# davide-gurrieri/parallel-GCN

Hardware: AMD Instinct MI355X
Metric: training epochs/sec (2-layer GCN, hidden=16) on reddit (higher is better)
Workload: dtype fp32

## Files before the change

include/pgcn.h:

```cpp
#ifndef PGCN_H
#define PGCN_H
#include <stddef.h>
#include <stdint.h>

#ifdef __cplusplus
extern "C" {
#endif

#define PGCN_OK 0
#define PGCN_E_INVALID (-1)
#define PGCN_E_NOMEM (-2)
#define PGCN_E_IO (-3)
#define PGCN_E_COMM (-4)
#define PGCN_E_NODEVICE (-5)

const char *pgcn_status_string(int status);
int pgcn_version(void);


void pgcn_rng_seed(uint64_t state[2]);
void pgcn_rng_seed_glibc(unsigned int seed, uint64_t state[2]);
void pgcn_rng_jump(uint64_t state[2], uint64_t k);

typedef struct pgcn_graph pgcn_graph;
// ... 227 lines not shown
#define PGCN_CKPT_ATTENTION 8
int pgcn_checkpoint_attention(const char *path, int *heads, float *dropout);
#define PGCN_CKPT_SAGE 16
int pgcn_checkpoint_sage(const char *path, int *aggregator, int *root_weight);
#define PGCN_CKPT_READOUT 32
int pgcn_checkpoint_readout(const char *path, int *mode, int *num_graphs);
#define PGCN_CKPT_LINKS 64
int pgcn_checkpoint_links(const char *path, int *decoder, long long *num_pairs);
int pgcn_params_sizeof(void);
long long pgcn_gcn_predict(pgcn_gcn *g, int *cls, float *conf, float *probs);
int pgcn_gcn_confusion(pgcn_gcn *g, int split, long long *counts);
long long pgcn_gcn_predict_multilabel(pgcn_gcn *g, uint32_t *bits, float *probs);
int pgcn_gcn_multilabel_counts(pgcn_gcn *g, int split, long long *counts);
long long pgcn_gcn_predict_links(pgcn_gcn *g, float *scores, float *probs);
int pgcn_gcn_link_counts(pgcn_gcn *g, int split, long long *counts);
int pgcn_gcn_score_pairs(pgcn_gcn *g, const int *src, const int *dst, long long m, float *scores);
int pgcn_gcn_profile(pgcn_gcn *g, int enable);
int pgcn_gcn_profile_read(pgcn_gcn *g, double *graphsum_ms_total, long long *graphsum_calls,
                          double *graphsum_bytes_total);
int pgcn_gcn_profile_read_mm(pgcn_gcn *g, double *ms_total, long long *calls,
                             double *flops_total);
int pgcn_gcn_node_range(pgcn_gcn *g, int *first, int *last);

typedef struct pgcn_dataset pgcn_dataset;
int pgcn_dataset_load(const char *root, const char *name, pgcn_dataset **out);
int pgcn_dataset_load_cached(const char *root, const char *name, pgcn_dataset **out,
                             int *from_cache);
int pgcn_dataset_save(const pgcn_dataset *ds, const char *path);
int pgcn_dataset_binarize(pgcn_dataset *ds);
int pgcn_dataset_load_binary(const char *path, pgcn_dataset **out);
int pgcn_dataset_synthetic(int n, int f, int c, long long undirected_edges, uint64_t seed,
                           pgcn_dataset **out);
int pgcn_dataset_set_multilabel(pgcn_dataset *ds, const uint32_t *bits, int words, int c);
int pgcn_dataset_load_labels(pgcn_dataset *ds, const char *path, int num_classes);
int pgcn_dataset_set_graphs(pgcn_dataset *ds, const int *graph_ptr, const int *label,
                            const int *split, int G, int num_classes);
int pgcn_dataset_load_graphs(pgcn_dataset *ds, const char *path, int num_classes);
int pgcn_dataset_set_links(pgcn_dataset *ds, const int *src, const int *dst, const int *label,
                           const int *split, long long E, int embed_dim);
int pgcn_dataset_load_links(pgcn_dataset *ds, const char *path, int embed_dim);
int pgcn_dataset_view(const pgcn_dataset *ds, pgcn_data *view, int *input_dim, int *output_dim);
int pgcn_dataset_free(pgcn_dataset *ds);

int pgcn_partition_bounds(int n, const int *indptr, int world, int *bounds_out, int *maxrows);
long long pgcn_partition_subgraph(int n, const int *indptr, const int *indices, int world,
                                  int rank, int *sub_indptr, int *sub_indices, float *sub_vals);

int pgcn_debug_rank_graph(int n, const int *indptr, const int *indices, int world, int rank,
                          int chunks, int chunk, pgcn_graph **out, int *rows, int *cols);
int pgcn_debug_set(const char *key, int value);
int pgcn_debug_knob(int index, const char **name, int *default_value);
int pgcn_debug_lds_check(int n_rows, int n_cols, const int *indptr, const int *indices,
                         int window, double *max_rel_err, long long *n_blocks);
long long pgcn_debug_lds_counts(int n_rows, int n_cols, const int *indptr, const int *indices,
                                int window, unsigned short *dst, long long cap, int *shape5);
long long pgcn_debug_path_count(const char *name, int reset);
int pgcn_debug_empty_launches(int n, void *stream);
int pgcn_debug_exp_check(const float *x, long long n, float *mine, float *lib, void *stream);
int pgcn_debug_div_check(const float *a, const float *b, long long n, float *q, void *stream);

typedef struct {
  const float *w;
  long long n_w;
  float wd;
  float *out2;
  const int *ctr;
  int ring_cap;
  float *sums;
  unsigned int *ticket;
  void *part4;
  int group;
  unsigned int *gticket;
  void *gpart4;
} pgcn_xent_final;
int pgcn_debug_ring_slice_rows(void);
int pgcn_debug_xent_fwd(float *logits, int ld, float *grad, const int *truth, int n, int c,
                        int count, int training, float *partials, int write_back,
                        const pgcn_xent_final *fin, void *stream);
int pgcn_debug_out_xent(const float *H, int ldh, int kh, const float *W, int ldw, float *logits,
                        int ld, float *grad, const int *truth, int n, int c, int count,
                        int training, float *partials, float *dH, int lddh, float *dWp,
                        float *table, const float *scale, const int *pos, int table_rows,
                        const pgcn_xent_final *fin, void *stream);
int pgcn_debug_finalize_ring(const float *partials, int n_blocks, int count, const float *w_l2,
                             long long n_l2, float weight_decay, float *out2, const int *ctr,
                             int ring_cap, float *sums, void *stream);
size_t pgcn_debug_tn_reduce_blocks_workspace(int n_blocks, int K, int ldp);
int pgcn_debug_tn_reduce_blocks(float *partial, int n_blocks, int K, int N, int ldp, float *C,
                                int ldc, void *stream);
int pgcn_debug_tn_reduce_one_pass(const float *partial, int n, int K, int N, int ldp, float *C,
                                  int ldc, void *stream);
int pgcn_debug_gemm_nib(int M, int N, int K, const float *A, int lda, const float *B, int ldb,
                        int trans_b, float *C, int ldc, const uint64_t *a_mask,
                        long long mask_base, long long mask_ld, float a_scale,
                        const uint64_t *mask_nib, void *stream);
int pgcn_debug_gemm_tn_nib(int M, int N, int K, const float *A, int lda, const float *G, int ldg,
                           float *C, int ldc, const uint64_t *a_mask, long long mask_base,
                           long long mask_ld, float a_scale, const uint64_t *mask_nib,
                           void *workspace, void *stream);
int pgcn_debug_spmm_csr(int m, int p, int ldc, const int *indptr, const int *indices,
                        const float *a, const uint64_t *mask, long long mask_base, float scale,
                        const float *b, float *c, float *c2, void *stream);
int pgcn_debug_spmm_csc_bwd(int nf, int p, int ldg, const int *csc_ptr, const int *csc_row,
                            const int *csc_pos, const float *a, const uint64_t *mask,
                            long long mask_base, float scale, const float *cgrad, float *bgrad,
                            long long nnz, const int *order, int tree, void *stream);
int pgcn_debug_dropout_mask(uint64_t *states, long long n_chunks, long long elem0,
                            long long elem_end, float p, uint64_t *mask, const void *table,
                            int per, int max_blocks, void *stream);
int pgcn_debug_dropout_mask2(uint64_t *states0, long long n_chunks0, long long elem0_0,
                             long long elem_end0, float p0, uint64_t *mask0, int per0,
                             uint64_t *states1, long long n_chunks1, long long elem0_1,
                             long long elem_end1, float p1, uint64_t *mask1, int per1,
                             const void *table, void *stream);
int pgcn_debug_dropout_apply(float *x, long long n, const uint64_t *mask, long long base,
                             float scale, void *stream);

#ifdef __cplusplus
}
#endif
#endif
```

parallel-gcn_amd/__init__.py:

```python
import ctypes
import os

import numpy as np

HERE = os.path.dirname(os.path.abspath(__file__))
LIB_PATH = os.environ.get("PGCN_LIB") or os.path.join(HERE, "libpgcn.so")

PGCN_OK = 0
PGCN_E_INVALID = -1
PGCN_E_NOMEM = -2
PGCN_E_IO = -3
PGCN_E_COMM = -4
PGCN_E_NODEVICE = -5
MAX_LAYERS = 16
PGCN_LOAD_WEIGHTS_ONLY = 1
PREDICT_ROWS = 64

if not os.path.exists(LIB_PATH):
    raise ImportError(f"{LIB_PATH} is not built: run `make -C parallel-gcn_amd` "
                      "(or __graft_entry__.build()); there is no fallback path")
lib = ctypes.CDLL(LIB_PATH)

c_int, c_ll, c_float, c_void_p = ctypes.c_int, ctypes.c_longlong, ctypes.c_float, ctypes.c_void_p
c_size_t, c_u64, c_double = ctypes.c_size_t, ctypes.c_uint64, ctypes.c_double
# ... 130 lines not shown
_sig("pgcn_finalize", c_int, c_void_p, c_int, c_int, c_void_p, c_ll, c_float, c_void_p, c_void_p)
_sig("pgcn_adam", c_int, c_void_p, c_void_p, c_void_p, c_void_p, c_ll, c_float, c_float, c_float,
     c_float, c_float, c_int, c_void_p)
_sig("pgcn_adam_step_size", c_float, c_float, c_float, c_float, c_int)
_sig("pgcn_params_default", None, P(PgcnParams))
_sig("pgcn_gcn_create", c_int, P(PgcnParams), P(PgcnData), c_int, P(c_void_p))
_sig("pgcn_comm_unique_id", c_int, c_void_p)
_sig("pgcn_gcn_create_dist", c_int, P(PgcnParams), P(PgcnData), c_int, c_int, c_int, c_void_p,
     P(c_void_p))
_sig("pgcn_gcn_destroy", c_int, c_void_p)
ALLGATHER_FN = ctypes.CFUNCTYPE(c_int, c_void_p, ctypes.c_size_t, c_void_p, c_void_p)
_sig("pgcn_gcn_create_peer", c_int, P(PgcnParams), P(PgcnData), c_int, c_int, c_int,
     ALLGATHER_FN, c_void_p, P(c_void_p))
_sig("pgcn_loopback_create", c_int, c_int, P(c_void_p))
_sig("pgcn_debug_gcn_create_solo", c_int, P(PgcnParams), P(PgcnData), c_int, c_int, c_int,
     P(c_void_p))
_sig("pgcn_loopback_destroy", c_int, c_void_p)
_sig("pgcn_gcn_create_loopback", c_int, P(PgcnParams), P(PgcnData), c_int, c_int, c_void_p,
     P(c_void_p))
_sig("pgcn_gcn_query", c_ll, c_void_p, ctypes.c_char_p)
_sig("pgcn_gcn_train_epoch", c_int, c_void_p, P(c_float))
_sig("pgcn_gcn_eval", c_int, c_void_p, c_int, P(c_float))
_sig("pgcn_gcn_epoch_async", c_int, c_void_p)
_sig("pgcn_gcn_sync", c_int, c_void_p)
_sig("pgcn_gcn_results", c_int, c_void_p, c_int, P(c_float))
_sig("pgcn_gcn_run", c_int, c_void_p, c_int)
_sig("pgcn_gcn_get_var", c_ll, c_void_p, c_int, c_int, P(c_float))
_sig("pgcn_gcn_num_vars", c_int, c_void_p)
_sig("pgcn_gcn_set_var", c_int, c_void_p, c_int, c_int, c_void_p, c_ll)
_sig("pgcn_gcn_save", c_int, c_void_p, ctypes.c_char_p)
_sig("pgcn_gcn_load", c_int, c_void_p, ctypes.c_char_p, c_int)
_sig("pgcn_checkpoint_info", c_int, ctypes.c_char_p, P(c_ll))
_sig("pgcn_checkpoint_flags", c_int, ctypes.c_char_p)
_sig("pgcn_checkpoint_attention", c_int, ctypes.c_char_p, P(c_int), P(c_float))
_sig("pgcn_checkpoint_sage", c_int, ctypes.c_char_p, P(c_int), P(c_int))
_sig("pgcn_checkpoint_readout", c_int, ctypes.c_char_p, P(c_int), P(c_int))
_sig("pgcn_checkpoint_links", c_int, ctypes.c_char_p, P(c_int), P(c_ll))
_sig("pgcn_gcn_predict_links", c_ll, c_void_p, c_void_p, c_void_p)
_sig("pgcn_gcn_link_counts", c_int, c_void_p, c_int, c_void_p)
_sig("pgcn_gcn_score_pairs", c_int, c_void_p, c_void_p, c_void_p, c_ll, c_void_p)
_sig("pgcn_dataset_set_links", c_int, c_void_p, c_void_p, c_void_p, c_void_p, c_void_p, c_ll, c_int)
_sig("pgcn_dataset_load_links", c_int, c_void_p, ctypes.c_char_p, c_int)
_sig("pgcn_gcn_predict", c_ll, c_void_p, c_void_p, c_void_p, c_void_p)
_sig("pgcn_gcn_confusion", c_int, c_void_p, c_int, c_void_p)
_sig("pgcn_predict_rows", c_int, c_void_p, c_int, c_int, c_int, c_void_p, c_void_p, c_void_p,
     c_int, c_void_p)
_sig("pgcn_confusion", c_int, c_void_p, c_void_p, c_int, c_int, c_void_p, c_void_p)
_sig("pgcn_bce_fwd", c_int, c_void_p, c_int, c_void_p, c_void_p, c_void_p, c_int, c_int, c_int,
     c_int, c_int, c_void_p, c_void_p)
_sig("pgcn_predict_multilabel_rows", c_int, c_void_p, c_int, c_int, c_int, c_void_p, c_int,
     c_void_p, c_int, c_void_p)
_sig("pgcn_multilabel_counts", c_int, c_void_p, c_void_p, c_void_p, c_int, c_int, c_int, c_void_p,
     c_void_p)
_sig("pgcn_gcn_predict_multilabel", c_ll, c_void_p, c_void_p, c_void_p)
_sig("pgcn_gcn_multilabel_counts", c_int, c_void_p, c_int, c_void_p)
_sig("pgcn_dataset_set_multilabel", c_int, c_void_p, c_void_p, c_int, c_int)
_sig("pgcn_dataset_load_labels", c_int, c_void_p, ctypes.c_char_p, c_int)
_sig("pgcn_dataset_set_graphs", c_int, c_void_p, c_void_p, c_void_p, c_void_p, c_int, c_int)
_sig("pgcn_dataset_load_graphs", c_int, c_void_p, ctypes.c_char_p, c_int)
_sig("pgcn_gcn_profile", c_int, c_void_p, c_int)
_sig("pgcn_gcn_profile_read", c_int, c_void_p, P(c_double), P(c_ll), P(c_double))
_sig("pgcn_gcn_profile_read_mm", c_int, c_void_p, P(c_double), P(c_ll), P(c_double))
_sig("pgcn_gcn_node_range", c_int, c_void_p, P(c_int), P(c_int))
_sig("pgcn_dataset_load", c_int, ctypes.c_char_p, ctypes.c_char_p, P(c_void_p))
_sig("pgcn_dataset_load_cached", c_int, ctypes.c_char_p, ctypes.c_char_p, P(c_void_p), P(c_int))
_sig("pgcn_dataset_save", c_int, c_void_p, ctypes.c_char_p)
_sig("pgcn_dataset_binarize", c_int, c_void_p)
_sig("pgcn_dataset_load_binary", c_int, ctypes.c_char_p, P(c_void_p))
_sig("pgcn_dataset_synthetic", c_int, c_int, c_int, c_int, c_ll, c_u64, P(c_void_p))
_sig("pgcn_dataset_view", c_int, c_void_p, P(PgcnData), P(c_int), P(c_int))
_sig("pgcn_dataset_free", c_int, c_void_p)
_sig("pgcn_debug_set", c_int, ctypes.c_char_p, c_int)
_sig("pgcn_debug_knob", c_int, c_int, ctypes.POINTER(ctypes.c_char_p), ctypes.POINTER(c_int))
_sig("pgcn_debug_path_count", c_ll, ctypes.c_char_p, c_int)
_sig("pgcn_debug_empty_launches", c_int, c_int, c_void_p)
_sig("pgcn_debug_exp_check", c_int, c_void_p, c_ll, c_void_p, c_void_p, c_void_p)
_sig("pgcn_debug_div_check", c_int, c_void_p, c_void_p, c_ll, c_void_p, c_void_p)
_sig("pgcn_debug_ring_slice_rows", c_int)
_sig("pgcn_debug_xent_fwd", c_int, c_void_p, c_int, c_void_p, c_void_p, c_int, c_int, c_int,
     c_int, c_void_p, c_int, P(PgcnXentFinal), c_void_p)
_sig("pgcn_debug_out_xent", c_int, c_void_p, c_int, c_int, c_void_p, c_int, c_void_p, c_int,
     c_void_p, c_void_p, c_int, c_int, c_int, c_int, c_void_p, c_void_p, c_int, c_void_p,
     c_void_p, c_void_p, c_void_p, c_int, P(PgcnXentFinal), c_void_p)
_sig("pgcn_debug_finalize_ring", c_int, c_void_p, c_int, c_int, c_void_p, c_ll, c_float,
     c_void_p, c_void_p, c_int, c_void_p, c_void_p)
_sig("pgcn_debug_tn_reduce_blocks_workspace", c_size_t, c_int, c_int, c_int)
_sig("pgcn_debug_tn_reduce_blocks", c_int, c_void_p, c_int, c_int, c_int, c_int, c_void_p, c_int,
     c_void_p)
_sig("pgcn_debug_tn_reduce_one_pass", c_int, c_void_p, c_int, c_int, c_int, c_int, c_void_p,
     c_int, c_void_p)
_sig("pgcn_debug_gemm_nib", c_int, c_int, c_int, c_int, c_void_p, c_int, c_void_p, c_int, c_int,
     c_void_p, c_int, c_void_p, c_ll, c_ll, c_float, c_void_p, c_void_p)
_sig("pgcn_debug_gemm_tn_nib", c_int, c_int, c_int, c_int, c_void_p, c_int, c_void_p, c_int,
     c_void_p, c_int, c_void_p, c_ll, c_ll, c_float, c_void_p, c_void_p, c_void_p)
_sig("pgcn_debug_spmm_csr", c_int, c_int, c_int, c_int, c_void_p, c_void_p, c_void_p, c_void_p,
     c_ll, c_float, c_void_p, c_void_p, c_void_p, c_void_p)
_sig("pgcn_debug_spmm_csc_bwd", c_int, c_int, c_int, c_int, c_void_p, c_void_p, c_void_p,
     c_void_p, c_void_p, c_ll, c_float, c_void_p, c_void_p, c_ll, c_void_p, c_int, c_void_p)
_sig("pgcn_debug_dropout_mask", c_int, c_void_p, c_ll, c_ll, c_ll, c_float, c_void_p, c_void_p,
     c_int, c_int, c_void_p)
_sig("pgcn_debug_dropout_mask2", c_int, c_void_p, c_ll, c_ll, c_ll, c_float, c_void_p, c_int,
     c_void_p, c_ll, c_ll, c_ll, c_float, c_void_p, c_int, c_void_p, c_void_p)
_sig("pgcn_debug_dropout_apply", c_int, c_void_p, c_ll, c_void_p, c_ll, c_float, c_void_p)
_sig("pgcn_debug_lds_check", c_int, c_int, c_int, c_void_p, c_void_p, c_int, P(ctypes.c_double),
     P(c_ll))
_sig("pgcn_debug_lds_counts", c_ll, c_int, c_int, c_void_p, c_void_p, c_int, c_void_p, c_ll,
     c_void_p)
_sig("pgcn_partition_bounds", c_int, c_int, c_void_p, c_int, c_void_p, P(c_int))
_sig("pgcn_debug_rank_graph", c_int, c_int, c_void_p, c_void_p, c_int, c_int, c_int, c_int,
     c_void_p, c_void_p, c_void_p)
_sig("pgcn_partition_subgraph", c_ll, c_int, c_void_p, c_void_p, c_int, c_int, c_void_p,
     c_void_p, c_void_p)


class PgcnError(RuntimeError):
    def __init__(self, status, where=""):
        self.status = status
        super().__init__(f"{where}: {lib.pgcn_status_string(status).decode()} ({status})")


def check(status, where=""):
    if status != PGCN_OK:
        raise PgcnError(status, where)
    return status


def _ptr(a):
    return a.ctypes.data_as(c_void_p)


KERNEL_PATHS = ("xs_nn_ring", "xs_tn_ring", "xs_nn", "xs_tn", "gs_ring", "gs_gather", "out_xent",
                "gemm_nn", "gemm_tn", "gemm_nn_w", "gemm_tn_w", "gat_fwd", "gat_bwd", "gat_heads",
                "spmm_csr", "spmm_csr_dual", "spmm_csc_256", "spmm_csc_1024", "spmm_tree_256",
                "spmm_tree_1024", "launches", "link_fwd", "link_bwd")


def path_counts(reset=False, thread=False):
    out = {}
    t = 2 if thread else 0
    for k in KERNEL_PATHS:
        n = lib.pgcn_debug_path_count(k.encode(), t)
        if n < 0:
            raise PgcnError(int(n), "path_count " + k)
        out[k] = int(n)
    if reset:
        lib.pgcn_debug_path_count(None, 1 | t)
    return out


def reset_path_counts(thread=False):
    check(int(lib.pgcn_debug_path_count(None, 3 if thread else 1)), "path_count reset")


class Dataset:

    def __init__(self, handle):
        self._h = c_void_p(handle)
        self._refresh()

    def _refresh(self):
        self.view = PgcnData()
        fi, fo = c_int(), c_int()
        check(lib.pgcn_dataset_view(self._h, ctypes.byref(self.view), ctypes.byref(fi),
                                    ctypes.byref(fo)), "dataset_view")
        self.input_dim, self.output_dim = fi.value, fo.value
        self.num_nodes = self.view.num_nodes
        n = self.num_nodes

        def arr(p, count, dt):
            if count == 0:
                return np.zeros(0, dt)
            return np.ctypeslib.as_array(ctypes.cast(p, P(ctypes.c_int if dt == np.int32 else c_float)),
                                         shape=(count,))
        self.graph_indptr = arr(self.view.graph_indptr, n + 1, np.int32)
        self.graph_indices = arr(self.view.graph_indices, int(self.graph_indptr[-1]), np.int32)
        self.feat_indptr = arr(self.view.feat_indptr, n + 1, np.int32)
        nnzx = int(self.feat_indptr[-1])
        self.feat_indices = arr(self.view.feat_indices, nnzx, np.int32)
        self.feat_values = arr(self.view.feat_values, nnzx, np.float32)
        self.label = arr(self.view.label, n, np.int32)
        self.split = arr(self.view.split, n, np.int32)
        self.label_words = self.view.label_words
        self.label_bits = None
        if self.view.label_bits and self.label_words:
            self.label_bits = np.ctypeslib.as_array(self.view.label_bits,
                                                    shape=(n, self.label_words))

        self.num_graphs = self.view.num_graphs
        self.graph_ptr = self.graph_label = self.graph_split = None
        if self.num_graphs > 0 and self.view.graph_ptr:
            g = self.num_graphs
            self.graph_ptr = arr(self.view.graph_ptr, g + 1, np.int32)
            self.graph_label = arr(self.view.graph_label, g, np.int32)
            self.graph_split = arr(self.view.graph_split, g, np.int32)

        self.num_pairs = self.view.num_pairs
        self.pair_src = self.pair_dst = self.pair_label = self.pair_split = None
        if self.num_pairs > 0 and self.view.pair_src:
            e = self.num_pairs
            self.pair_src = arr(self.view.pair_src, e, np.int32)
            self.pair_dst = arr(self.view.pair_dst, e, np.int32)
            self.pair_label = arr(self.view.pair_label, e, np.int32)
            self.pair_split = arr(self.view.pair_split, e, np.int32)

    def set_links(self, src, dst, labels, splits, embed_dim):
        a = [np.ascontiguousarray(x, np.int32) for x in (src, dst, labels, splits)]
        if a[0].ndim != 1 or any(x.shape != a[0].shape for x in a):
            raise ValueError("set_links: src, dst, labels, splits [E]")
        check(lib.pgcn_dataset_set_links(self._h, *(_ptr(x) for x in a), a[0].size, embed_dim),
              "dataset_set_links")
        self._refresh()

    def load_links(self, path, embed_dim):
        check(lib.pgcn_dataset_load_links(self._h, os.fsencode(path), embed_dim),
              f"dataset_load_links {path}")
        self._refresh()

# ... 531 lines not shown

def rng_jump(state, k):
    s = (c_u64 * 2)(int(state[0]), int(state[1]))
    lib.pgcn_rng_jump(s, int(k))
    return np.array([s[0], s[1]], np.uint64)


def rng_jump_table(period):
    t = np.zeros(16 * 256 * 2, np.uint64)
    check(lib.pgcn_rng_jump_table(int(period), _ptr(t)), "rng_jump_table")
    return t


def partition_bounds(indptr, world):
    indptr = np.ascontiguousarray(indptr, np.int32)
    b = np.zeros(world + 1, np.int32)
    mr = c_int()
    check(lib.pgcn_partition_bounds(len(indptr) - 1, _ptr(indptr), world, _ptr(b),
                                    ctypes.byref(mr)), "partition_bounds")
    return b, mr.value


def partition_subgraph(indptr, indices, world, rank):
    indptr = np.ascontiguousarray(indptr, np.int32)
    indices = np.ascontiguousarray(indices, np.int32)
    n = len(indptr) - 1
    _, maxrows = partition_bounds(indptr, world)
    nnz = lib.pgcn_partition_subgraph(n, _ptr(indptr), _ptr(indices), world, rank, None, None, None)
    if nnz < 0:
        raise PgcnError(int(nnz), "partition_subgraph")
    sp = np.zeros(world * maxrows + 1, np.int32)
    si = np.zeros(max(nnz, 1), np.int32)
    sv = np.zeros(max(nnz, 1), np.float32)
    lib.pgcn_partition_subgraph(n, _ptr(indptr), _ptr(indices), world, rank, _ptr(sp), _ptr(si),
                                _ptr(sv))
    return sp, si[:nnz], sv[:nnz]


def csr_transpose(indptr, indices, n_cols):
    indptr = np.ascontiguousarray(indptr, np.int32)
    indices = np.ascontiguousarray(indices, np.int32)
    m, nnz = len(indptr) - 1, int(indptr[-1])
    cp = np.zeros(n_cols + 1, np.int32)
    cr = np.zeros(max(nnz, 1), np.int32)
    cpos = np.zeros(max(nnz, 1), np.int32)
    check(lib.pgcn_csr_transpose(m, n_cols, _ptr(indptr), _ptr(indices), _ptr(cp), _ptr(cr),
                                 _ptr(cpos)), "csr_transpose")
    return cp, cr[:nnz], cpos[:nnz]


EXPORTED = [
    "pgcn_status_string", "pgcn_version", "pgcn_rng_seed", "pgcn_rng_seed_glibc", "pgcn_rng_jump",
    "pgcn_graph_create", "pgcn_graph_create_values", "pgcn_debug_rank_graph",
    "pgcn_graph_destroy", "pgcn_graph_nnz", "pgcn_graphsum", "pgcn_gemm", "pgcn_gemm_tn_workspace",
    "pgcn_gemm_tn", "pgcn_mask_nibbles", "pgcn_gemm_xstream", "pgcn_gemm_xstream_dual",
    "pgcn_gemm_tn_xstream", "pgcn_gemm_xstream_flat", "pgcn_gemm_tn_xstream_flat",
    "pgcn_spmm_csr", "pgcn_spmm_csc_bwd", "pgcn_csr_transpose",
    "pgcn_rng_jump_table", "pgcn_dropout_mask", "pgcn_dropout_apply", "pgcn_relu_fwd",
    "pgcn_relu_bwd", "pgcn_residual_fwd", "pgcn_residual_bwd", "pgcn_params_sizeof",
    "pgcn_layernorm_fwd", "pgcn_layernorm_bwd_workspace", "pgcn_layernorm_bwd",
    "pgcn_debug_layernorm_fwd_tail",
    "pgcn_gat_scores", "pgcn_gat_fwd", "pgcn_gat_bwd_workspace", "pgcn_gat_bwd",
    "pgcn_gat_scores_mh", "pgcn_gat_fwd_mh", "pgcn_gat_bwd_workspace_mh", "pgcn_gat_bwd_mh",
    "pgcn_graph_create_mean", "pgcn_agg_max_fwd", "pgcn_agg_max_bwd",
    "pgcn_checkpoint_flags", "pgcn_checkpoint_attention", "pgcn_checkpoint_sage", "pgcn_xent_blocks", "pgcn_xent_fwd", "pgcn_finalize", "pgcn_adam",
    "pgcn_adam_step_size", "pgcn_params_default", "pgcn_gcn_create", "pgcn_comm_unique_id",
    "pgcn_gcn_create_dist", "pgcn_gcn_create_peer", "pgcn_loopback_create",
    "pgcn_loopback_destroy",
    "pgcn_debug_gcn_create_solo",
    "pgcn_gcn_create_loopback", "pgcn_gcn_query", "pgcn_gcn_destroy", "pgcn_gcn_train_epoch", "pgcn_gcn_eval",
    "pgcn_gcn_epoch_async", "pgcn_gcn_sync", "pgcn_gcn_results", "pgcn_gcn_run",
    "pgcn_gcn_get_var", "pgcn_gcn_num_vars", "pgcn_gcn_profile", "pgcn_gcn_profile_read",
    "pgcn_gcn_set_var", "pgcn_gcn_save", "pgcn_gcn_load", "pgcn_checkpoint_info",
    "pgcn_gcn_predict", "pgcn_gcn_confusion", "pgcn_predict_rows", "pgcn_confusion",
    "pgcn_gcn_profile_read_mm",
    "pgcn_gcn_node_range", "pgcn_dataset_load", "pgcn_dataset_load_cached", "pgcn_dataset_save",
    "pgcn_dataset_load_binary", "pgcn_dataset_binarize", "pgcn_dataset_synthetic",
    "pgcn_dataset_view",
    "pgcn_dataset_free", "pgcn_partition_bounds", "pgcn_partition_subgraph", "pgcn_debug_set",
    "pgcn_debug_knob",
    "pgcn_debug_lds_check", "pgcn_debug_lds_counts", "pgcn_debug_path_count",
    "pgcn_debug_empty_launches", "pgcn_debug_exp_check", "pgcn_debug_div_check",
    "pgcn_debug_ring_slice_rows", "pgcn_debug_xent_fwd", "pgcn_debug_out_xent",
    "pgcn_debug_finalize_ring", "pgcn_debug_tn_reduce_blocks_workspace",
    "pgcn_debug_tn_reduce_blocks", "pgcn_debug_tn_reduce_one_pass",
    "pgcn_debug_gemm_nib", "pgcn_debug_gemm_tn_nib",
    "pgcn_debug_spmm_csr", "pgcn_debug_spmm_csc_bwd", "pgcn_debug_dropout_mask",
    "pgcn_debug_dropout_mask2", "pgcn_debug_dropout_apply",
    "pgcn_bce_fwd", "pgcn_predict_multilabel_rows", "pgcn_multilabel_counts",
    "pgcn_gcn_predict_multilabel", "pgcn_gcn_multilabel_counts", "pgcn_dataset_set_multilabel",
    "pgcn_dataset_load_labels",
    "pgcn_readout_chunk_rows", "pgcn_readout_workspace", "pgcn_readout_fwd", "pgcn_readout_bwd",
    "pgcn_dataset_set_graphs", "pgcn_dataset_load_graphs", "pgcn_checkpoint_readout",
    "pgcn_links_create", "pgcn_links_destroy", "pgcn_link_segment_slots", "pgcn_links_slots",
    "pgcn_link_score_fwd", "pgcn_link_score_bwd", "pgcn_debug_links_incidence",
    "pgcn_checkpoint_links", "pgcn_gcn_predict_links", "pgcn_gcn_link_counts",
    "pgcn_gcn_score_pairs", "pgcn_dataset_set_links", "pgcn_dataset_load_links",
]
```

parallel-gcn_amd/csrc/capi.cpp:

```cpp
#include <atomic>
#include <climits>
#include <cstring>
#include <memory>

#include "../../include/pgcn.h"
#include "common.hpp"
#include "host/checkpoint.hpp"
#include "host/comm.hpp"
#include "host/data.hpp"
#include "host/gcn.hpp"
#include "host/graph.hpp"
#include "kernels.hpp"
#include "knobs.hpp"
#include "rng.hpp"

#include <cmath>

using namespace pgcn;

namespace pgcn {
namespace {
std::atomic<long long> g_path_hits[KP_COUNT];
thread_local long long t_path_hits[KP_COUNT];
const char *const kPathNames[KP_COUNT] = {"xs_nn_ring", "xs_tn_ring", "xs_nn",   "xs_tn",
                                          "gs_ring",    "gs_gather",  "out_xent", "gemm_nn",
                                          "gemm_tn",    "gemm_nn_w",  "gemm_tn_w", "gat_fwd",
                                          "gat_bwd",    "gat_heads",  "spmm_csr",
                                          "spmm_csr_dual", "spmm_csc_256", "spmm_csc_1024",
                                          "spmm_tree_256", "spmm_tree_1024", "launches",
                                          "link_fwd",   "link_bwd"};
}
void note_path(KernelPath p) {
  g_path_hits[p].fetch_add(1, std::memory_order_relaxed);
  t_path_hits[p]++;
}
}

struct pgcn_graph {
  std::unique_ptr<DevGraph> g;
};
struct pgcn_links {
  std::unique_ptr<LinkIndexDev> l;
};
struct pgcn_gcn {
  std::unique_ptr<GCN> g;
};
struct pgcn_dataset {
  GCNData d;
};
struct pgcn_loopback {
  std::shared_ptr<LoopbackGroup> g;
};

namespace {
void check_device() {
  int n = 0;
  if (hipGetDeviceCount(&n) != hipSuccess || n <= 0)
    throw Error(PGCN_E_NODEVICE, "no HIP device visible: the engine has no CPU fallback");
}

void refuse_single_gpu_only(const pgcn_params *p) {
  PGCN_CHECK(!p->attention, PGCN_E_INVALID,
             "attention: single GPU only (edge-cut attention is not supported)");
  PGCN_CHECK(!p->aggregator && !p->root_weight, PGCN_E_INVALID,
             "aggregator: single GPU only (edge-cut SAGE layers are not supported)");
  PGCN_CHECK(!p->readout, PGCN_E_INVALID,
             "readout: single GPU only (edge-cut graph classification is not supported)");
  PGCN_CHECK(!p->link_decoder, PGCN_E_INVALID,
             "link_decoder: single GPU only (edge-cut link prediction is not supported)");
}

GCNParams to_params(const pgcn_params *p, const pgcn_data *d) {
  GCNParams q;
  q.num_nodes = d->num_nodes;
  q.input_dim = p->input_dim;
  q.output_dim = p->output_dim;
  q.n_layers = p->n_layers;
  q.hidden_dims.assign(p->hidden_dims, p->hidden_dims + std::max(0, p->n_layers - 1));
  q.dropouts.assign(p->dropouts, p->dropouts + std::max(0, p->n_layers));
  q.epochs = p->epochs;
  q.early_stopping = p->early_stopping;
  q.reassociate_last = p->reassociate_last != 0;
  q.seed = p->seed;
  q.residual = p->residual != 0;
  q.layer_norm = p->layer_norm != 0;
  q.multilabel = p->multilabel != 0;
  q.attention = p->attention != 0;
  q.attention_heads = p->attention_heads == 0 ? 1 : p->attention_heads;
  q.attention_dropout = p->attention_dropout;
  PGCN_CHECK(p->root_weight == 0 || p->root_weight == 1, PGCN_E_INVALID,
             "root_weight must be 0 or 1");
  q.aggregator = p->aggregator;
  q.root_weight = p->root_weight != 0;
  PGCN_CHECK(p->readout >= kReadoutNone && p->readout <= kReadoutMax, PGCN_E_INVALID,
             "readout must be 0 (none), 1 (sum), 2 (mean) or 3 (max)");
  PGCN_CHECK(!p->readout || !p->multilabel, PGCN_E_INVALID,
             "readout cannot be combined with multilabel");
  q.readout = p->readout;
  PGCN_CHECK(p->link_decoder == 0 || p->link_decoder == 1, PGCN_E_INVALID,
             "link_decoder must be 0 (none) or 1 (dot product)");
  PGCN_CHECK(!p->link_decoder || (!p->multilabel && !p->readout), PGCN_E_INVALID,
             "link_decoder cannot be combined with multilabel or readout");
  q.link_decoder = p->link_decoder;
  return q;
}
AdamParams to_adam(const pgcn_params *p) {
  AdamParams a;
  a.learning_rate = p->learning_rate;
  a.weight_decay = p->weight_decay;
  a.beta1 = p->beta1;
  a.beta2 = p->beta2;
  a.eps = p->eps;
  return a;
// ... 1456 lines not shown
}

namespace {
void check_final(const pgcn_xent_final *f, const char *what) {
  if (!f) return;
  PGCN_CHECK(f->ticket && f->part4 && f->out2, PGCN_E_INVALID, what);
  PGCN_CHECK(f->group >= 0 && (f->group == 0 || (f->gticket && f->gpart4)), PGCN_E_INVALID, what);
  PGCN_CHECK(f->n_w >= 0 && (f->n_w == 0 || f->w) && (!f->ctr || f->ring_cap >= 1),
             PGCN_E_INVALID, what);
}
XentFinal to_final(const pgcn_xent_final &f) {
  XentFinal x;
  x.w = f.w;
  x.n_w = f.n_w;
  x.wd = f.wd;
  x.out2 = f.out2;
  x.ctr = f.ctr;
  x.ring_cap = f.ctr ? f.ring_cap : 1;
  x.sums = f.sums;
  x.ticket = f.ticket;
  x.part4 = static_cast<float4 *>(f.part4);
  x.group = f.group;
  x.gticket = f.gticket;
  x.gpart4 = static_cast<float4 *>(f.gpart4);
  return x;
}
}

extern "C" {

int pgcn_debug_ring_slice_rows(void) { return RING_SR; }

int pgcn_debug_xent_fwd(float *logits, int ld, float *grad, const int *truth, int n, int c,
                        int count, int training, float *partials, int write_back,
                        const pgcn_xent_final *fin, void *stream) {
  return guarded([&] {
    PGCN_CHECK(n >= 0 && c >= 1 && c <= ld && ld <= 124 && ld % 4 == 0 && count >= 0,
               PGCN_E_INVALID, "debug_xent_fwd: 1 <= c <= ld <= 124, ld % 4 == 0");
    PGCN_CHECK(n == 0 || (logits && truth && partials && (grad || !training)), PGCN_E_INVALID,
               "debug_xent_fwd: null argument");
    check_final(fin, "debug_xent_fwd: the finish needs its ticket, partials and output");
    if (n == 0) return;
    XentFinal xf;
    if (fin) xf = to_final(*fin);
    launch_xent_fwd(logits, ld, grad, truth, n, c, count, training, partials, as_stream(stream),
                    write_back != 0, fin ? &xf : nullptr);
    PGCN_HIP(hipGetLastError());
  });
}

int pgcn_debug_out_xent(const float *H, int ldh, int kh, const float *W, int ldw, float *logits,
                        int ld, float *grad, const int *truth, int n, int c, int count,
                        int training, float *partials, float *dH, int lddh, float *dWp,
                        float *table, const float *scale, const int *pos, int table_rows,
                        const pgcn_xent_final *fin, void *stream) {
  return guarded([&] {
    PGCN_CHECK(n >= 0 && kh >= 1 && kh <= 16 && ldh >= kh, PGCN_E_INVALID,
               "debug_out_xent: 1 <= kh <= 16, ldh >= kh");
    PGCN_CHECK(c >= 1 && c <= ld && ld <= 116 && ld % 4 == 0 && ldw >= c && count >= 0,
               PGCN_E_INVALID, "debug_out_xent: 1 <= c <= ld <= 116, ld % 4 == 0, ldw >= c");
    PGCN_CHECK(!dH || lddh >= kh, PGCN_E_INVALID, "debug_out_xent: lddh >= kh");
    PGCN_CHECK(!dWp || ld <= 48, PGCN_E_INVALID,
               "debug_out_xent: the weight-grad partial needs <= 48 classes");
    PGCN_CHECK(!table || (kh == 16 && scale && dH && (pos || table_rows >= 0)), PGCN_E_INVALID,
               "debug_out_xent: a prescaled table of a 16-column dH");
    PGCN_CHECK(n == 0 || (H && W && logits && truth && partials && (grad || !training)),
               PGCN_E_INVALID, "debug_out_xent: null argument");
    check_final(fin, "debug_out_xent: the finish needs its ticket, partials and output");
    if (n == 0) return;
    XentFinal xf;
    if (fin) xf = to_final(*fin);
    XentTable tb;
    tb.table = table;
    tb.scale = scale;
    tb.pos = pos;
    tb.rows = table_rows;
    launch_out_xent(H, ldh, kh, W, ldw, logits, ld, grad, truth, n, c, count, training, partials,
                    as_stream(stream), dH, lddh, dWp, table ? &tb : nullptr,
                    fin ? &xf : nullptr);
    PGCN_HIP(hipGetLastError());
  });
}

int pgcn_debug_finalize_ring(const float *partials, int n_blocks, int count, const float *w_l2,
                             long long n_l2, float weight_decay, float *out2, const int *ctr,
                             int ring_cap, float *sums, void *stream) {
  return guarded([&] {
    PGCN_CHECK(n_blocks >= 0 && n_l2 >= 0 && (n_l2 == 0 || w_l2) && (!ctr || ring_cap >= 1),
               PGCN_E_INVALID, "debug_finalize_ring args");
    PGCN_CHECK(n_blocks == 0 || (partials && out2), PGCN_E_INVALID,
               "debug_finalize_ring: null argument");
    if (n_blocks == 0) return;
    launch_reduce_scalars(partials, n_blocks, w_l2, n_l2, sums, as_stream(stream), count,
                          weight_decay, out2, ctr, ctr ? ring_cap : 1);
    PGCN_HIP(hipGetLastError());
  });
}

size_t pgcn_debug_tn_reduce_blocks_workspace(int n_blocks, int K, int ldp) {
  if (n_blocks < 0 || K < 1 || ldp < 1) return 0;
  return tn_reduce_blocks_workspace(n_blocks, K, ldp);
}

int pgcn_debug_tn_reduce_blocks(float *partial, int n_blocks, int K, int N, int ldp, float *C,
                                int ldc, void *stream) {
  return guarded([&] {
    PGCN_CHECK(n_blocks >= 0 && K >= 1 && N >= 1 && N <= ldc && ldc <= ldp, PGCN_E_INVALID,
               "debug_tn_reduce_blocks: K >= 1, 1 <= N <= ldc <= ldp");
    PGCN_CHECK(n_blocks == 0 || (partial && C), PGCN_E_INVALID,
               "debug_tn_reduce_blocks: null argument");
    if (n_blocks == 0) return;
    launch_tn_reduce_blocks(partial, n_blocks, K, N, ldp, C, ldc, as_stream(stream));
    PGCN_HIP(hipGetLastError());
  });
}

int pgcn_debug_tn_reduce_one_pass(const float *partial, int n, int K, int N, int ldp, float *C,
                                  int ldc, void *stream) {
  return guarded([&] {
    PGCN_CHECK(n >= 0 && K >= 1 && N >= 1 && N <= ldc && ldc <= ldp, PGCN_E_INVALID,
               "debug_tn_reduce_one_pass: K >= 1, 1 <= N <= ldc <= ldp");
    PGCN_CHECK(n == 0 || (partial && C), PGCN_E_INVALID,
               "debug_tn_reduce_one_pass: null argument");
    if (n == 0) return;
    launch_tn_reduce_one_pass(partial, n, K, N, ldp, C, ldc, as_stream(stream));
    PGCN_HIP(hipGetLastError());
  });
}

int pgcn_debug_gemm_nib(int M, int N, int K, const float *A, int lda, const float *B, int ldb,
                        int trans_b, float *C, int ldc, const uint64_t *a_mask,
                        long long mask_base, long long mask_ld, float a_scale,
                        const uint64_t *mask_nib, void *stream) {
  return guarded([&] {
    PGCN_CHECK(A && B && C && M >= 0 && K > 0 && ldc >= N, PGCN_E_INVALID, "debug_gemm_nib args");
    launch_gemm_nn(M, N, K, A, lda, B, ldb, trans_b, C, ldc, a_mask, mask_base, mask_ld, a_scale,
                   as_stream(stream), mask_nib);
    PGCN_HIP(hipGetLastError());
  });
}

int pgcn_debug_gemm_tn_nib(int M, int N, int K, const float *A, int lda, const float *G, int ldg,
                           float *C, int ldc, const uint64_t *a_mask, long long mask_base,
                           long long mask_ld, float a_scale, const uint64_t *mask_nib,
                           void *workspace, void *stream) {
  return guarded([&] {
    PGCN_CHECK(A && G && C && workspace && K > 0 && ldc >= N, PGCN_E_INVALID,
               "debug_gemm_tn_nib args");
    launch_gemm_tn(M, N, K, A, lda, G, ldg, C, ldc, a_mask, mask_base, mask_ld, a_scale,
                   workspace, as_stream(stream), mask_nib);
    PGCN_HIP(hipGetLastError());
  });
}

int pgcn_debug_spmm_csr(int m, int p, int ldc, const int *indptr, const int *indices,
                        const float *a, const uint64_t *mask, long long mask_base, float scale,
                        const float *b, float *c, float *c2, void *stream) {
  return guarded([&] {
    PGCN_CHECK(m >= 0 && p >= 1 && ldc >= p && mask_base >= 0, PGCN_E_INVALID,
               "debug_spmm_csr: m >= 0, 1 <= p <= ldc, mask_base >= 0");
    PGCN_CHECK(m == 0 || (indptr && indices && a && b && c), PGCN_E_INVALID,
               "debug_spmm_csr: null argument");
    if (c2)
      launch_spmm_csr_dual(m, p, ldc, indptr, indices, a, mask, mask_base, scale, b, c, c2,
                           as_stream(stream));
    else
// ... 109 lines not shown
```

parallel-gcn_amd/csrc/host/gcn.cpp:

```cpp
#include "gcn.hpp"

#include <algorithm>
#include <chrono>
#include <cmath>
#include <cstdio>
#include <cstring>

#include "../kernels.hpp"
#include "../rng.hpp"
#include "checkpoint.hpp"

namespace pgcn {

constexpr int kFinishMaxBlocks = 512, kFinishGroup = 64;
constexpr int kMmSideRows = 65536;

Adam::Adam(const std::vector<shared_ptr<Variable>> &weights, const std::vector<bool> &decays,
           const AdamParams &p)
    : params(p) {
  PGCN_CHECK(weights.size() == decays.size(), PGCN_E_INVALID,
             "Adam: weights and decays must have the same size");
  for (size_t i = 0; i < weights.size(); i++) {
    Var v;
    v.w = weights[i];
// ... 705 lines not shown
  if (knobs_.fuse_epilogue & kFuseMatmulTails) fuse_matmul_tails();
  if (knobs_.co_draw && dropouts_.size() >= 2 && (knobs_.co_draw == 2 || !feats.dense) &&
      dropouts_[0] && dropouts_[1])
    const_cast<Dropout *>(dropouts_[0])->co_draw = dropouts_[1];
  if (knobs_.fuse_output && !params.multilabel && !head_rows()) fuse_output_layer();
  optimizer = Adam(weights, decays, adam_params);
  prepare_graphs();
  build_eval_ax();
  const auto *pc = dynamic_cast<const PeerComm *>(comm.get());
  if (knobs_.eval_tail && pc && !pc->host_ordered() && comm->world() > 1) {
    for (int i = 0; i < (int)modules.size(); i++)
      if (dynamic_cast<const GraphSum *>(modules[(size_t)i].get())) tail_gs = i;
    ctx.tail_fork = Event::create();
    ctx.tail_done = Event::create();
  }
  PGCN_HIP(hipDeviceSynchronize());
  if (comm) comm->host_barrier();
}

void GCN::build_eval_ax() {
  Event ax0 = Event::create(true), ax1 = Event::create(true);
  if (feats.ax && !comm) {
    graph->prepare(16);
    ax0.record(stream.get());
    for (int c0 = 0; c0 < feats.cols; c0 += 16) {
      const int c = std::min(c0, feats.ldx - 16);
      graph->graphsum(feats.x.get() + c, feats.ldx, feats.ax.get() + c, feats.ldx, 16, stream.get());
    }
    ax1.record(stream.get());
    stream.sync();
    PGCN_HIP(hipEventElapsedTime(&ax_build_ms, ax0.get(), ax1.get()));
  }
  if (feats.ax && comm) {
    const int h = part.chunk_rows(), nk = (int)chunk_graphs.size();
    DeviceBuffer<float> partial((size_t)part.world * h * 16), own((size_t)nk * h * 16);
    for (auto &gk : chunk_graphs) gk->prepare(16);
    comm->host_barrier();
    ax0.record(stream.get());
    for (int c0 = 0; c0 < feats.cols; c0 += 16) {
      const int c = std::min(c0, feats.ldx - 16);
      for (int k = 0; k < nk; k++) {
        chunk_graphs[(size_t)k]->graphsum(feats.x.get() + c, feats.ldx, partial.get(), 16, 16,
                                          stream.get());
        comm->reduce_scatter_sum(partial.get(), own.get() + (size_t)k * h * 16, (size_t)h * 16,
                                 stream.get());
      }
      PGCN_HIP(hipMemcpy2DAsync(feats.ax.get() + c, sizeof(float) * feats.ldx, own.get(),
                                sizeof(float) * 16, sizeof(float) * 16, (size_t)part.local_rows(),
                                hipMemcpyDeviceToDevice, stream.get()));
    }
    ax1.record(stream.get());
    stream.sync();
    PGCN_HIP(hipEventElapsedTime(&ax_build_ms, ax0.get(), ax1.get()));
  }
}

void GCN::prepare_graphs() {
  for (int split = 1; split <= 2; split++) {
    set_split(split);
    for (const auto &m : modules) {
      const auto *gs = dynamic_cast<const GraphSum *>(m.get());
      if (!gs) continue;
      const int d = gs->width();
      for (DevGraph *g : {gs->forward_graph(), gs->backward_graph()})
        if (g) g->prepare(d);
      for (DevGraph *g : ctx.chunk_graphs) g->prepare(d);
      for (DevGraph *g : ctx.chunk_split_graphs) g->prepare(d);
      for (DevGraph *g : ctx.chunk_col_graphs) g->prepare(d);
    }
  }
  set_split(1);
}

void GCN::fuse_output_layer() {
  const size_t n = modules.size();
  if (n < 2) return;
  auto *ce = dynamic_cast<CrossEntropyLoss *>(modules[n - 1].get());
  auto *mm = dynamic_cast<Matmul *>(modules[n - 2].get());
  if (!ce || !mm || mm->output() != ce->input() || mm->inner() > 16 || mm->inner() < 1) return;
  if (ce->input()->ld > 116 || mm->input()->rows != ce->input()->rows) return;
  ce->fused = mm;
  mm->fused_forward = true;
  auto *gs = n >= 3 ? dynamic_cast<GraphSum *>(modules[n - 3].get()) : nullptr;
  if (gs && gs->output() == mm->input()) ce->dh_reader = gs;
}

void GCN::fuse_epilogues() {
  const size_t n = modules.size();
  for (size_t i = 0; i < n; i++) {
    if (auto *ln = dynamic_cast<LayerNorm *>(modules[i].get())) {
      const Variable *v = ln->variable();
      auto *relu = i + 1 < n ? dynamic_cast<ReLU *>(modules[i + 1].get()) : nullptr;
      if (!relu || relu->variable() != v || v->ld != v->cols) continue;
      ln->fwd_relu = relu;
      auto *res = i + 2 < n ? dynamic_cast<ResidualConnection *>(modules[i + 2].get()) : nullptr;
      if (res && res->current() == v && res->previous()->ld == v->ld) ln->fwd_res = res;
      const size_t di = i + (ln->fwd_res ? 3 : 2);
      auto *drop = di < n ? dynamic_cast<Dropout *>(modules[di].get()) : nullptr;
      if (res && !ln->fwd_res) drop = nullptr;
      if (drop && drop->variable() == v) ln->fwd_drop = drop;
      continue;
    }
    auto *gs = dynamic_cast<GraphSum *>(modules[i].get());
    if (!gs) continue;
    const Variable *out = gs->output(), *in = gs->input();
    if (i + 1 < n && out->ld == out->cols) {
      auto *relu = dynamic_cast<ReLU *>(modules[i + 1].get());
      if (relu && relu->variable() == out) {
        gs->fwd_relu = relu;
        auto *res = i + 2 < n ? dynamic_cast<ResidualConnection *>(modules[i + 2].get()) : nullptr;
        if (res && res->current() == out && res->previous()->ld == out->ld) gs->fwd_res = res;
        const size_t di = i + (gs->fwd_res ? 3 : 2);
        auto *drop = di < n ? dynamic_cast<Dropout *>(modules[di].get()) : nullptr;
        if (res && !gs->fwd_res) drop = nullptr;
        if (drop && drop->variable() == out) gs->fwd_drop = drop;
        fused_tails_++;
        const size_t k = di + (gs->fwd_drop ? 1 : 0);
        auto *next = k < n ? dynamic_cast<GraphSum *>(modules[k].get()) : nullptr;
        if (next && next->input() == out) gs->fwd_next = next;
      }
    }
    if (i >= 1 && in->ld == in->cols) {
      auto *drop = dynamic_cast<Dropout *>(modules[i - 1].get());
      const bool has_drop = drop && drop->variable() == in;
      size_t ri = has_drop ? i - 2 : i - 1;
      auto *res = ri < n ? dynamic_cast<ResidualConnection *>(modules[ri].get()) : nullptr;
      if (res && res->current() == in) ri--;
      auto *relu = ri < n ? dynamic_cast<ReLU *>(modules[ri].get()) : nullptr;
      if (relu && relu->variable() == in) {
        gs->bwd_relu = relu;
        if (has_drop) gs->bwd_drop = drop;
        fused_tails_++;
        auto *next = ri >= 1 ? dynamic_cast<GraphSum *>(modules[ri - 1].get()) : nullptr;
        if (next && next->output() == in) gs->bwd_next = next;
      }
    }
  }
}

void GCN::fuse_matmul_tails() {
  const size_t n = modules.size();
  for (size_t i = 1; i < n; i++) {
    auto *mm = dynamic_cast<Matmul *>(modules[i].get());
    if (!mm || mm->input()->ld != mm->input()->cols) continue;
    const Variable *a = mm->input(), *c = mm->output();
    if (!xstream_ok(a->cols, c->cols) || xstream_ring_ok(c->cols, c->ld)) continue;
    if (a->skip_from || a->dev_grad_z) continue;
    auto *drop = dynamic_cast<Dropout *>(modules[i - 1].get());
    if (drop && drop->variable() != a) drop = nullptr;
    const size_t ri = drop ? i - 2 : i - 1;
    auto *relu = ri < n ? dynamic_cast<ReLU *>(modules[ri].get()) : nullptr;
    if (!relu || relu->variable() != a) continue;
    bool taken = false;
    for (auto &m : modules) {
      auto *gs = dynamic_cast<GraphSum *>(m.get());
      if (gs && gs->bwd_relu == relu) taken = true;
    }
    if (taken) continue;
    mm->bwd_relu = relu;
    mm->bwd_drop = drop;
    fused_tails_++;
  }
}

void GCN::insert_first_layer() {
  const int prow = part.maxrows, h = params.hidden_dims.front();
  auto drop = std::make_unique<Dropout>(nullptr, params.dropouts.front(), rngs[0], &ctx);
// ... 986 lines not shown
```

parallel-gcn_amd/csrc/host/graph.cpp:

```cpp
#include "graph.hpp"

#include <atomic>

#include <algorithm>
#include <climits>
#include <cmath>
#include <functional>
#include <numeric>
#include <thread>

namespace pgcn {

float graph_coef(int deg_src, int deg_dst) {
  return (float)(1.0 / (double)sqrtf((float)(deg_src * deg_dst)));
}

void parallel_for(long long n, const std::function<void(long long, long long)> &f, int threads,
                  long long min_parallel) {
  if (threads <= 0) {
    threads = (int)std::thread::hardware_concurrency();
    if (threads > 16) threads = 16;
    if (threads < 1) threads = 1;
  }
  if (n < min_parallel || threads == 1) {
// ... 489 lines not shown
}

float *DevGraph::table_wide(size_t floats) {
  DevGraph *o = table_owner_ ? table_owner_ : this;
  if (!o->lds_) o->build_lds();
  if (o->lds_->tables.size() < floats) o->lds_->tables.allocate(floats);
  return o->lds_->tables.get();
}

void DevGraph::graphsum(const float *in, int ld_in, float *out, int ld_out, int dim,
                        hipStream_t s, bool compact_in, const GsEpilogue *epi, bool prestaged,
                        bool tables_ready, const PeerSink *push, hipStream_t tail_st,
                        hipEvent_t fork) {
  const int *col_map = compact_in ? nullptr : col_map_.get();
  PGCN_CHECK(ld_in % 4 == 0 && ld_out % 4 == 0 && ld_in >= dim && ld_out >= dim,
             PGCN_E_INVALID, "graphsum: leading dims must be multiples of 4 and >= dim");
  PGCN_CHECK(!epi || epi->mode == 0 || epilogue_ok(dim, ld_in, ld_out), PGCN_E_INVALID,
             "graphsum: epilogue on a multi-pass width");
  PGCN_CHECK(!prestaged || uses_lds(dim), PGCN_E_INVALID, "graphsum: prestaged input, plain path");
  if (uses_lds(dim)) {
    if (!lds_) build_lds();
    const int ldm = std::min(ld_in, ld_out);
    PGCN_CHECK(!prestaged || dim <= 16, PGCN_E_INVALID,
               "graphsum: prestaged input on a path without a ring table");
    const size_t table = (size_t)ceil_div(n_cols_, RING_SR) * RING_SR * 16;
    const int n_pass = ceil_div(dim, 16);
    PGCN_CHECK(!tail_st || (push && n_pass == 1), PGCN_E_INVALID,
               "graphsum: a tail stream for a one-pass push only");
    auto pass_col = [&](int p) { return std::min(16 * p, ldm - 16); };
    const bool batch = n_pass > 1 && !col_map && ld_in <= 128;
    PGCN_CHECK(!tables_ready || (can_share_tables(dim, ld_in) && (n_pass == 1 || batch)),
               PGCN_E_INVALID, "graphsum: shared tables on a call that prescales per pass");
    RingPasses ps;
    if (batch) {
      PGCN_CHECK(n_pass <= 8, PGCN_E_INVALID, "graphsum: batched passes");
      for (int p = 0; p < n_pass; p++) ps.c[ps.n++] = pass_col(p);
    }
    float *tables = batch ? table_wide(table * n_pass) : nullptr;
    if (batch && !tables_ready)
      launch_ring_prescale_wide(lds_->s, in, ld_in, std::min(ld_in, ps.c[ps.n - 1] + 16), ps,
                                tables, (long long)table, s);
    for (int p = 0; p < n_pass; p++) {
      const int c = pass_col(p);
      GsEpilogue ep = epi ? *epi : GsEpilogue{};
      ep.col0 = c;
      PeerSink pk;
      if (push) {
        pk = *push;
        for (int q = 0; q < pk.world; q++) pk.dst[q] += c;
        pk.slot_bytes -= 4LL * c;
        pk.signal = p == n_pass - 1 ? push->signal : 0;
      }
      launch_graphsum_ring(lds_->s, in + c, ld_in, out ? out + c : nullptr, ld_out,
                           batch ? tables + table * p : table_scratch(), lds_->partial.get(), s,
                           col_map, &ep, prestaged || batch || tables_ready, push ? &pk : nullptr,
                           tail_st, fork);
    }
    return;
  }
  PGCN_CHECK(!push, PGCN_E_INVALID, "graphsum: push on the plain path");
  if (dim > 16 && !graphsum_vec_supported((dim + 3) / 4)) {
    const int ldm = std::min(ld_in, ld_out);
    for (int c0 = 0; c0 < dim; c0 += 16) {
      const int c = std::min(c0, ldm - 16);
      graphsum(in + c, ld_in, out + c, ld_out, 16, s, compact_in);
    }
    return;
  }
  const int vec = (dim + 3) / 4;
  Sched &sc = schedule(vec);
  const bool blocked = sc.s.nbc > 1;
  const bool orig = col_map && !blocked && knobs_.gs_orig_cols;
  if (col_map && !orig) {
    const size_t need = (size_t)n_cols_ * ld_in;
    if (col_in_.size() < need) col_in_.allocate(need);
    launch_gather_rows(in, col_map, n_cols_, ld_in, col_in_.get(), s);
    in = col_in_.get();
  }
  launch_graphsum(sc.s, blocked ? bindices_.get() : (orig ? orig_indices_.get() : indices_.get()),
                  blocked ? bvals_.get() : vals_.get(), in, ld_in, out, ld_out, sc.partial.get(), s,
                  epi);
}

static void gat_segments(int n, const std::vector<int> &ptr, std::vector<int4> *segs,
                         std::vector<int2> *longs) {
  for (int i = 0; i < n; i++) {
    const int b = ptr[(size_t)i], e = ptr[(size_t)i + 1];
    if (e - b <= kGatSeg) continue;
    const int first = (int)segs->size();
    if (longs) longs->push_back(make_int2(i, first));
    for (int s = b; s < e; s += kGatSeg)
      segs->push_back(make_int4(i, s, std::min(s + kGatSeg, e), first));
  }
}

const GatPattern &DevGraph::gat_pattern() {
  if (gat_) return gat_->p;
  PGCN_CHECK(n_rows_ == n_cols_, PGCN_E_INVALID, "graph attention needs a square pattern");
  auto g = std::make_unique<GatDev>();
  const int n = n_rows_;
  std::vector<int> cptr((size_t)n + 1, 0), crow((size_t)nnz_), cpos((size_t)nnz_);
  for (long long k = 0; k < nnz_; k++) {
    const int j = h_indices_[(size_t)k];
    PGCN_CHECK(j >= 0 && j < n, PGCN_E_INVALID, "graph attention: column id out of range");
    cptr[(size_t)j + 1]++;
  }
  for (int j = 0; j < n; j++) cptr[(size_t)j + 1] += cptr[(size_t)j];
  std::vector<int> fill(cptr.begin(), cptr.end() - 1);
  for (int i = 0; i < n; i++) {
    PGCN_CHECK(h_indptr_[(size_t)i] <= h_indptr_[(size_t)i + 1], PGCN_E_INVALID,
               "graph attention: indptr must not decrease");
    for (int k = h_indptr_[(size_t)i]; k < h_indptr_[(size_t)i + 1]; k++) {
      const int o = fill[(size_t)h_indices_[(size_t)k]]++;
      crow[(size_t)o] = i;
      cpos[(size_t)o] = k;
    }
  }
  std::vector<int4> rsegs, csegs;
  std::vector<int2> lcols;
  gat_segments(n, h_indptr_, &rsegs, nullptr);
  gat_segments(n, cptr, &csegs, &lcols);
  auto up = [](auto &buf, const auto &host) {
    buf.allocate(std::max<size_t>(host.size(), 1));
    if (!host.empty()) buf.upload(host);
  };
  up(g->indptr, h_indptr_);
  up(g->csc_ptr, cptr);
  up(g->csc_row, crow);
  up(g->csc_pos, cpos);
  up(g->row_segs, rsegs);
  up(g->col_segs, csegs);
  up(g->long_cols, lcols);
  g->row_ws.allocate(std::max<size_t>(rsegs.size() * kGatWsStride, 4));
  g->row_ws.zero();
  GatPattern &p = g->p;
  p.n = n;
  p.nnz = nnz_;
  p.indptr = g->indptr.get();
  p.indices = indices_.get();
  p.csc_ptr = g->csc_ptr.get();
  p.csc_row = g->csc_row.get();
  p.csc_pos = g->csc_pos.get();
  p.n_row_segs = (int)rsegs.size();
  p.n_col_segs = (int)csegs.size();
  p.n_long_cols = (int)lcols.size();
  p.row_segs = g->row_segs.get();
  p.col_segs = g->col_segs.get();
  p.long_cols = g->long_cols.get();
  p.row_ws = g->row_ws.get();
  gat_ = std::move(g);
  return gat_->p;
}

std::unique_ptr<DevGraph> make_mean_graph(int n, const int *indptr, const int *indices,
                                          bool transpose, const Knobs &knobs) {
  const int nnz = indptr[n];
  std::vector<float> inv((size_t)n, 0.0f), one((size_t)n, 1.0f);
  for (int i = 0; i < n; i++)
    if (indptr[i + 1] > indptr[i]) inv[(size_t)i] = 1.0f / (float)(indptr[i + 1] - indptr[i]);
  std::vector<float> vals((size_t)std::max(nnz, 1));
  std::unique_ptr<DevGraph> g;
  if (!transpose) {
    for (int i = 0; i < n; i++)
      for (int k = indptr[i]; k < indptr[i + 1]; k++) vals[(size_t)k] = inv[(size_t)i];
    g = std::make_unique<DevGraph>(n, n, indptr, indices, vals.data(), knobs);
    g->set_scales(std::move(inv), std::move(one));
// ... 112 lines not shown
```

parallel-gcn_amd/csrc/host/graph.hpp:

```cpp
#pragma once
#include <functional>
#include <map>
#include <memory>
#include <vector>

#include "../kernels.hpp"
#include "../knobs.hpp"
#include "runtime.hpp"

namespace pgcn {

float graph_coef(int deg_src, int deg_dst);

std::vector<float> graph_coefs(int n, const int *indptr, const int *indices);

void parallel_for(long long n, const std::function<void(long long, long long)> &f,
                  int threads = 0, long long min_parallel = 100000);

bool csr_symmetric(int n, const int *indptr, const int *indices);

std::vector<float> degree_scales(int n, const int *indptr);

struct LdsHost {
  int n_batches = 0, t_max = 0, n_blocks = 4, ns = LDS_SLOTS;
  bool pair = false;
  int w = RING_W;
  std::vector<int> nsl;
  std::vector<int2> slices;
  std::vector<int> rows;
  std::vector<unsigned short> counts;
  std::vector<long long> wave_off;
  std::vector<unsigned short> entries;
};
std::vector<int> column_cuts(int n_cols, const std::vector<int> &indices,
                             int n_blocks = kGraphBlocks);
int lds_blocks(int n_rows, int n_cols, const Knobs &k);
int lds_slots(int n_rows, int n_cols);
std::vector<int> ring_cuts(int n_cols, const std::vector<int> &indices, int n_blocks);
LdsHost build_ring_host(int n_rows, int n_cols, const std::vector<int> &indptr,
                        const std::vector<int> &indices, const std::vector<int> &bcut,
                        int ns = LDS_SLOTS, bool pair = false, int window = RING_W);
int ring_window_for(int n_rows, int n_cols, long long nnz, int n_blocks, const Knobs &k);
void ring_emulate(const LdsHost &h, int n_rows, const float *in, double *out);

class DevGraph;
std::unique_ptr<DevGraph> make_mean_graph(int n, const int *indptr, const int *indices,
                                          bool transpose, const Knobs &knobs = process_knobs());

class DevGraph {
 public:
  DevGraph(int n_rows, int n_cols, const int *indptr, const int *indices, const float *vals,
           const Knobs &knobs = process_knobs());
  int rows() const { return n_rows_; }
  int cols() const { return n_cols_; }
  long long nnz() const { return nnz_; }
  void graphsum(const float *in, int ld_in, float *out, int ld_out, int dim, hipStream_t s,
                bool compact_in = false, const GsEpilogue *epi = nullptr, bool prestaged = false,
                bool tables_ready = false, const PeerSink *push = nullptr,
                hipStream_t tail_st = nullptr, hipEvent_t fork = nullptr);
  void share_tables(DevGraph *owner);
  bool can_share_tables(int dim, int ld_in) const;
  const DevGraph *table_owner() const { return table_owner_; }
  float *ring_table(int dim, const float **next_scale);
  float *ring_table_mapped(int dim, const float **next_scale, const int **pos, int *pos_rows);
  bool epilogue_ok(int dim, int ld_in, int ld_out) const;
  bool uses_lds(int dim) const;
  void prepare(int dim);
  double algorithmic_bytes(int dim) const;
  int column_blocks(int dim);
  const GatPattern &gat_pattern();
  const SageWs &sage_ws();

  void set_scales(std::vector<float> row_scale, std::vector<float> col_scale);
  std::unique_ptr<DevGraph> row_subset(const std::vector<int> &rows) const;
  std::unique_ptr<DevGraph> col_subset(const std::vector<int> &cols) const;

  static constexpr int kBlocks = kGraphBlocks;
  static constexpr double kL2Budget = 4.0e6;
  static constexpr long long kSmallNnz = 1 << 20;
  static constexpr int kWideCap = 1536;
  static constexpr long long kLdsMinBytes = 1 << 20;
  static constexpr int kLdsMinRows = 32768;

 private:
  struct Sched {
    GraphSchedule s;
    DeviceBuffer<int4> items, comb, wide;
    DeviceBuffer<int> block_items, slot_comb, comb_ctr;
    DeviceBuffer<float> partial;
  };
  Sched &schedule(int vec);
  void build_blocked();
  void compute_cuts();
  void build_lds();
  struct LdsSched {
    LdsSchedule s;
    DeviceBuffer<uint2> entries;
    DeviceBuffer<long long> wave_off;
    DeviceBuffer<unsigned short> counts;
    DeviceBuffer<int2> slices;
    DeviceBuffer<int> n_slices, rows;
    DeviceBuffer<float> row_scale, col_scale, scratch, partial;
    DeviceBuffer<float> tables;
  };
  std::unique_ptr<LdsSched> lds_;
  struct GatDev {
    GatPattern p;
    DeviceBuffer<int> indptr, csc_ptr, csc_row, csc_pos;
    DeviceBuffer<int4> row_segs, col_segs;
    DeviceBuffer<int2> long_cols;
    DeviceBuffer<float> row_ws;
  };
  std::unique_ptr<GatDev> gat_;
  struct SageDev {
    SageWs w;
    DeviceBuffer<float> row_val, col_ws;
    DeviceBuffer<int> row_arg;
  };
  std::unique_ptr<SageDev> sage_;
  DevGraph *table_owner_ = nullptr;
  float *table_scratch();
  float *table_wide(size_t floats);
  std::vector<float> h_row_scale_, h_col_scale_;
  DeviceBuffer<int> col_map_;
  DeviceBuffer<int> col_pos_;
  int col_pos_rows_ = 0;
  DeviceBuffer<float> col_in_;
  DeviceBuffer<int> orig_indices_;
  int n_rows_, n_cols_;
  long long nnz_;
  const Knobs knobs_;
  std::vector<int> h_indptr_, h_indices_;
  std::vector<float> h_vals_;
  DeviceBuffer<int> indices_;
  DeviceBuffer<float> vals_;
  bool blocked_built_ = false;
  std::vector<int> bcut_;
  std::vector<int> lds_cut_;
  std::vector<long long> bseg_;
  long long bnnz_ = 0;
  DeviceBuffer<int> bindices_;
  DeviceBuffer<float> bvals_;
// ... 25 lines not shown
```

parallel-gcn_amd/csrc/host/module.cpp:

```cpp
#include "module.hpp"

#include <algorithm>
#include <utility>

#include "../kernels.hpp"

namespace pgcn {

namespace {
struct MmProfile {
  ModuleContext *ctx;
  hipStream_t s;
  double flops;
  Event e0, e1;
  MmProfile(ModuleContext *c, hipStream_t st, double f) : ctx(c), s(st), flops(f) {
    if (!on()) return;
    e0 = Event::create(true);
    e1 = Event::create(true);
    e0.record(s);
  }
  bool on() const { return ctx->profile && ctx->mm_events && flops > 0; }
  ~MmProfile() {
    if (!on()) return;
    e1.record(s);
// ... 440 lines not shown
                          s.get());
      bytes = sk->algorithmic_bytes(dim);
    }
    if (ctx->profile) e1.record(s.get());
  } else if (ctx->comm && mode != 1 && ctx->chunk_graphs.size() == 1 &&
             dynamic_cast<PeerComm *>(ctx->comm) && cgs[0]->uses_lds(dim)) {
    auto *pc = static_cast<PeerComm *>(ctx->comm);
    DevGraph *gk = cgs[0];
    const int h = out->rows;
    hipStream_t ts = s.get();
    if (ctx->tail_stream && dim <= 16) {
      ts = ctx->tail_stream;
      ctx->tail_used = true;
    }
    PeerSink k = pc->sink(h, (size_t)out->ld);
    pc->note((size_t)h * out->ld * ctx->comm->world() * sizeof(float), 1.0);
    gk->graphsum(src, in->ld, nullptr, out->ld, dim, s.get(), false, nullptr, prestaged, false, &k,
                 ts != s.get() ? ts : nullptr, ctx->tail_fork.get());
    bytes = gk->algorithmic_bytes(dim);
    pc->wait(ts);
    launch_gs_gather_finish(dst, out->ld, ctx->local_rows, (dim + 3) / 4 * 4,
                            epi && epi->mode ? *epi : GsEpilogue{}, pc->recv(), ts);
    if (ctx->profile) e1.record(ts);
  } else if (ctx->comm) {
    const size_t h = (size_t)out->rows / ctx->chunk_graphs.size();
    for (size_t k = 0; k < ctx->chunk_graphs.size(); k++) {
      if (mode == 1) {
        DevGraph *sk = ctx->chunk_split_graphs[k];
        if (sk->rows() > 0) {
          const size_t need = (size_t)sk->rows() * out->ld;
          if (compact.size() < need) compact.allocate(need);
          sk->graphsum(src, in->ld, compact.get(), out->ld, dim, s.get());
          launch_scatter_rows(compact.get(), ctx->chunk_split_rows[k], sk->rows(), out->ld,
                              partial[k].get(), s.get());
          bytes += sk->algorithmic_bytes(dim);
        }
      } else {
        DevGraph *gk = cgs[k];
        const bool shared = k > 0 && gk->table_owner() == cgs[0] && gk->can_share_tables(dim, in->ld);
        gk->graphsum(src, in->ld, partial[k].get(), out->ld, dim, s.get(), false, nullptr,
                     k == 0 && prestaged, shared);
        bytes += gk->algorithmic_bytes(dim);
      }
      if (ctx->chunk_graphs.size() == 1) {
        ctx->comm->reduce_scatter_sum(partial[k].get(), dst, h * out->ld, s.get());
        continue;
      }
      computed[k].record(s.get());
      computed[k].wait_on(ctx->comm_stream);
      ctx->comm->reduce_scatter_sum(partial[k].get(), dst + k * h * out->ld, h * out->ld,
                                    ctx->comm_stream);
    }
    if (ctx->chunk_graphs.size() > 1) {
      reduced.record(ctx->comm_stream);
      reduced.wait_on(s.get());
    }
    if (epi && epi->mode) launch_gs_finish(dst, out->ld, ctx->local_rows, dim, *epi, s.get());
    if (ctx->profile) e1.record(s.get());
  } else {
    graph->graphsum(src, in->ld, dst, out->ld, dim, s.get(), false, epi, prestaged);
    bytes = graph->algorithmic_bytes(dim);
    if (ctx->profile) e1.record(s.get());
  }
  if (ctx->profile) {
    ctx->gs_events->emplace_back(e0, e1);
    ctx->gs_bytes->push_back(bytes);
  }
}

void GraphSum::forward(bool training, const Stream &s) const {
  const bool pre = prestaged_fwd;
  prestaged_fwd = false;
  PGCN_CHECK(!pre || ((training || !first_layer) &&
                      !(last_layer && ctx->comm && !ctx->chunk_split_graphs.empty())),
             PGCN_E_INVALID, "graphsum: prestaged input on a path that does not read it");
  if (!training && first_layer) return;
  if (last_layer && ctx->comm && !ctx->chunk_split_graphs.empty()) {
    run(in->dev_data.get(), out->dev_data.get(), s, 1);
    return;
  }
  DevGraph *sg = last_layer && !ctx->comm ? ctx->split_graph : nullptr;
  if (!sg) {
    const GsEpilogue epi = forward_epilogue(training, s, graph);
    run(in->dev_data.get(), out->dev_data.get(), s, 0, &epi, pre);
    return;
  }
  float *dst;
  if (ctx->compact_n) {
    dst = ctx->compact_z->dev_data.get();
  } else {
    const size_t need = (size_t)std::max(sg->rows(), 1) * out->ld;
    if (compact.size() < need) compact.allocate(need);
    dst = compact.get();
  }
  Event e0, e1;
  if (ctx->profile) {
    e0 = Event::create(true);
    e1 = Event::create(true);
    e0.record(s.get());
  }
  sg->graphsum(in->dev_data.get(), in->ld, dst, out->ld, dim, s.get(), false, nullptr, pre);
  if (ctx->profile) {
    e1.record(s.get());
    ctx->gs_events->emplace_back(e0, e1);
    ctx->gs_bytes->push_back(sg->algorithmic_bytes(dim));
  }
  if (!ctx->compact_n)
    launch_scatter_rows(dst, ctx->split_rows, sg->rows(), out->ld, out->dev_data.get(), s.get());
}

void GraphSum::backward(const Stream &s) const {
  const bool pre = prestaged_bwd;
  prestaged_bwd = false;
  if (last_layer && ctx->comm && !ctx->chunk_col_graphs.empty()) {
    const GsEpilogue epi = backward_epilogue(ctx->chunk_col_graphs[0]);
    run(out->dev_grad.get(), backward_dst(epi), s, 2, &epi, pre);
    return;
  }
  DevGraph *cg = last_layer && !ctx->comm ? ctx->split_colgraph : nullptr;
  if (!cg) {
    const GsEpilogue epi = backward_epilogue(graph);
    const float *src = out->dev_grad_z ? out->dev_grad_z.get() : out->dev_grad.get();
    run(src, backward_dst(epi), s, 0, &epi, pre);
    return;
  }
  Event e0, e1;
  if (ctx->profile) {
    e0 = Event::create(true);
    e1 = Event::create(true);
    e0.record(s.get());
  }
  const float *g_in = ctx->compact_n ? ctx->compact_z->dev_grad.get() : out->dev_grad.get();
  const GsEpilogue epi = backward_epilogue(cg);
  cg->graphsum(g_in, out->ld, backward_dst(epi), in->ld, dim, s.get(), ctx->compact_n > 0, &epi,
               pre);
  if (ctx->profile) {
    e1.record(s.get());
    ctx->gs_events->emplace_back(e0, e1);
    ctx->gs_bytes->push_back(cg->algorithmic_bytes(dim));
  }
}

GraphAttention::GraphAttention(shared_ptr<Variable> in_, shared_ptr<Variable> out_,
                               DevGraph *graph_, int dim_, shared_ptr<Variable> attn_,
                               long long offset_, int heads_, float p_,
                               shared_ptr<DropoutRng> rng_, ModuleContext *ctx_)
    : in(std::move(in_)), out(std::move(out_)), attn(std::move(attn_)), graph(graph_), dim(dim_),
      offset(offset_), heads(heads_), p(p_), rng(std::move(rng_)), ctx(ctx_) {
  PGCN_CHECK(in && out && attn && graph && dim >= 1 && dim <= kGatMaxWidth && in->cols == dim &&
                 out->cols == dim && graph->rows() == graph->cols() && in->rows >= graph->rows() &&
                 out->rows >= graph->rows() && offset >= 0 && offset + 2LL * dim <= attn->size,
             PGCN_E_INVALID, "attention: widths up to 128 on a square pattern");
  PGCN_CHECK(gat_heads_ok(dim, heads) && heads <= kGatMaxHeads, PGCN_E_INVALID,
             "attention: heads must divide the width into head widths of 4, 8, 16, 32, 64 or 128");
  PGCN_CHECK(p >= 0.0f && p < 1.0f && (p > 0.0f) == (rng != nullptr) && (!rng || ctx),
             PGCN_E_INVALID, "attention: dropout in [0, 1), with its mask stream");
  const GatPattern &g = graph->gat_pattern();
  PGCN_CHECK(!rng || (rng->elem_begin == 0 && rng->elem_end == g.nnz * heads), PGCN_E_INVALID,
             "attention: the mask stream covers nnz * heads weights");
  u.allocate((size_t)std::max(g.n, 1) * heads);
  v.allocate((size_t)std::max(g.n, 1) * heads);
  alpha.allocate((size_t)std::max<long long>(g.nnz, 1) * heads);
  ws.allocate(std::max<size_t>(gat_bwd_workspace(g, dim, heads) / sizeof(float), 4));
  z.allocate((size_t)std::max(g.n, 1) * out->ld);
  for (const auto *b : {&u, &v, &alpha, &ws, &z}) b->zero();
}
// ... 254 lines not shown
void LayerNorm::backward(const Stream &s) const {
  if (!in->dev_grad || !norm->dev_grad) return;
  float *g = in->dev_grad_z ? in->dev_grad_z.get() : in->dev_grad.get();
  float *dgamma = norm->dev_grad.get() + offset;
  launch_layernorm_bwd(g, in->ld, xhat.get(), in->ld, rstd.get(), norm->dev_data.get() + offset,
                       rows, in->cols, g, in->ld, dgamma, dgamma + in->cols, ws.get(), s.get());
}

Matmul::Matmul(shared_ptr<Variable> a_, shared_ptr<Variable> b_, shared_ptr<Variable> c_,
               int m_, int n_, int p_, ModuleContext *ctx_)
    : a(std::move(a_)), b(std::move(b_)), c(std::move(c_)), m(m_), n(n_), p(p_), ctx(ctx_) {}

void Matmul::forward(bool training, const Stream &s) const {
  if (fused_forward && !(last_layer && ctx->compact_n)) return;
  const bool cmp = last_layer && ctx->compact_n;
  const Variable &A = cmp ? *ctx->compact_z : *a, &C = cmp ? *ctx->compact_out : *c;
  MmProfile prof(ctx, s.get(), 2.0 * (cmp ? ctx->compact_n : m) * p * n);
  launch_gemm_nn(cmp ? ctx->compact_n : m, p, n, A.dev_data.get(), A.ld, b->dev_data.get(), b->ld,
                 0, C.dev_data.get(), C.ld, nullptr, 0, 0, 1.0f, s.get());
}

void Matmul::backward_input(const Stream &s) const {
  launch_gemm_nn(m, n, p, c->dev_grad.get(), c->ld, b->dev_data.get(), b->ld, 1, a->dev_grad.get(),
                 a->ld, nullptr, 0, 0, 1.0f, s.get());
  add_skip_grad(s);
}

void Matmul::add_skip_grad(const Stream &s) const {
  if (!a->skip_from || !a->dev_grad) return;
  launch_residual_bwd(a->dev_grad.get(), a->skip_from->dev_grad.get(), (long long)m * a->ld,
                      s.get());
}

void Matmul::backward_weight(hipStream_t s, void *ws) const {
  launch_gemm_tn(m, p, n, a->dev_data.get(), a->ld, c->dev_grad.get(), c->ld, b->dev_grad.get(),
                 b->ld, nullptr, 0, 0, 1.0f, ws, s);
}

void Matmul::backward(const Stream &s) const {
  const bool cmp = last_layer && ctx->compact_n;
  const bool a_done = input_grad_done && !cmp;
  const bool b_done = weight_grad_done && !cmp;
  input_grad_done = weight_grad_done = false;
  const Variable &A = cmp ? *ctx->compact_z : *a, &C = cmp ? *ctx->compact_out : *c;
  const int rows = cmp ? ctx->compact_n : m;
  const bool side = ctx->mm_side && ctx->side_stream && ctx->gemm_workspace_side && !ctx->profile;
  MmProfile prof(ctx, s.get(), 2.0 * rows * p * n * ((a_done ? 0 : 1) + (side || b_done ? 0 : 1)));
  if (side) {
    ctx->mm_fork.record(s.get());
    ctx->mm_fork.wait_on(ctx->side_stream);
    launch_gemm_tn(rows, p, n, A.dev_data.get(), A.ld, C.dev_grad.get(), C.ld, b->dev_grad.get(),
                   b->ld, nullptr, 0, 0, 1.0f, ctx->gemm_workspace_side, ctx->side_stream);
    ctx->side_pending = true;
  }
  if (!a_done && bwd_relu && !cmp && !A.skip_from && !A.dev_grad_z && A.ld == n &&
      xstream_ok(n, p) && !xstream_ring_ok(p, C.ld)) {
    XsEpilogue e;
    if (bwd_drop) {
      e.bwd_drop = bwd_drop->state().mask.get();
      e.drop_base = bwd_drop->state().mask_base;
      e.drop_scale = bwd_drop->scale();
      bwd_drop->skip_backward = true;
    }
    e.bwd_relu = bwd_relu->mask_ptr();
    bwd_relu->skip_backward = true;
    launch_xstream_nn(rows, n, p, C.dev_grad.get(), C.ld, b->dev_data.get(), b->ld, 1,
                      A.dev_grad.get(), A.ld, nullptr, 1.0f, s.get(), nullptr, &e);
  } else if (!a_done) {
    launch_gemm_nn(rows, n, p, C.dev_grad.get(), C.ld, b->dev_data.get(), b->ld, 1,
                   A.dev_grad.get(), A.ld, nullptr, 0, 0, 1.0f, s.get());
  }
  if (!cmp) add_skip_grad(s);
  if (!side && !b_done)
    launch_gemm_tn(rows, p, n, A.dev_data.get(), A.ld, C.dev_grad.get(), C.ld, b->dev_grad.get(),
                   b->ld, nullptr, 0, 0, 1.0f, ctx->gemm_workspace, s.get());
}

CrossEntropyLoss::CrossEntropyLoss(shared_ptr<Variable> logits_, int num_classes_,
                                   ModuleContext *ctx_)
    : logits(std::move(logits_)), num_classes(num_classes_), ctx(ctx_) {}


void CrossEntropyLoss::forward(bool training, const Stream &s) const {
  if (fused && !ctx->compact_n) {
    const Variable &Hv = *fused->input(), &Wv = *fused->weight();
    const double mm = 2.0 * logits->rows * num_classes * fused->inner();
    MmProfile prof(ctx, s.get(), training ? 3.0 * mm : mm);
    float *dH = Hv.dev_grad ? Hv.dev_grad.get() : nullptr;
    const int nb = xent_blocks(logits->rows);
    float *dWp = nullptr;
    bool deferred = false;
    const Knobs &kn = *ctx->knobs;
    if (training && kn.fuse_output >= 2 &&
        (kn.fuse_output == 3 || logits->rows >= 65536 || ctx->comm) &&
        Wv.dev_grad && logits->ld <= 48 &&
        !ctx->mm_side &&
        tn_reduce_blocks_workspace(nb, fused->inner(), 48) <= ctx->gemm_workspace_bytes)
      dWp = static_cast<float *>(ctx->gemm_workspace);
    bool one_pass = false;
    if (training && !dWp && kn.fuse_output >= 2 && kn.defer_wgrad && !ctx->comm &&
        nb <= kDeferWgradMaxBlocks && Wv.dev_grad && logits->ld <= 48 && !ctx->mm_side) {
      dWp = tn_defer_blocks(nb, fused->inner(), num_classes, 48, Wv.dev_grad.get(), Wv.ld);
      deferred = dWp != nullptr;
      if (!dWp && (size_t)nb * fused->inner() * 48 * sizeof(float) <= ctx->gemm_workspace_bytes) {
        dWp = static_cast<float *>(ctx->gemm_workspace);
        one_pass = true;
      }
    }
    XentTable tb;
    const bool staged = training && dH && dh_reader && fused->inner() == 16 &&
                        dh_reader->claim_backward_table(Hv.rows, Hv.ld, &tb);
    launch_out_xent(Hv.dev_data.get(), Hv.ld, fused->inner(), Wv.dev_data.get(), Wv.ld,
                    logits->dev_data.get(), logits->ld, training ? logits->dev_grad.get() : nullptr,
                    ctx->truth, logits->rows, num_classes, ctx->count, training ? 1 : 0,
                    ctx->xent_partials, s.get(), dH, Hv.ld, dWp, staged ? &tb : nullptr, ctx->fin);
    ctx->fin_taken = ctx->fin != nullptr;
    if (one_pass)
      launch_tn_reduce_one_pass(dWp, nb, fused->inner(), num_classes, 48, Wv.dev_grad.get(),
                                Wv.ld, s.get());
    else if (dWp && !deferred)
      launch_tn_reduce_blocks(dWp, nb, fused->inner(), num_classes, 48, Wv.dev_grad.get(), Wv.ld,
                              s.get());
    fused->input_grad_done = training && dH;
    fused->weight_grad_done = dWp != nullptr;
    return;
  }
  const Variable &L = ctx->compact_n ? *ctx->compact_out : *logits;
  launch_xent_fwd(L.dev_data.get(), L.ld, training ? L.dev_grad.get() : nullptr,
                  ctx->compact_n ? ctx->compact_truth : ctx->truth,
                  ctx->compact_n ? ctx->compact_n : logits->rows, num_classes, ctx->count,
                  training ? 1 : 0, ctx->xent_partials, s.get(), ctx->compact_n ? 0 : 1,
                  ctx->fin);
  ctx->fin_taken = ctx->fin != nullptr;
}

void CrossEntropyLoss::backward(const Stream &) const {}

BCEWithLogitsLoss::BCEWithLogitsLoss(shared_ptr<Variable> logits_, int num_classes_,
                                     ModuleContext *ctx_)
    : logits(std::move(logits_)), num_classes(num_classes_), ctx(ctx_) {}

void BCEWithLogitsLoss::forward(bool training, const Stream &s) const {
  const bool cmp = ctx->compact_n != 0;
  const Variable &L = cmp ? *ctx->compact_out : *logits;
  PGCN_CHECK(ctx->label_bits && (!cmp || ctx->compact_label_bits), PGCN_E_INVALID,
             "BCEWithLogitsLoss: no label bits");
  launch_bce_fwd(L.dev_data.get(), L.ld, training ? L.dev_grad.get() : nullptr,
                 cmp ? ctx->compact_truth : ctx->truth,
                 cmp ? ctx->compact_label_bits : ctx->label_bits, ctx->label_words,
                 cmp ? ctx->compact_n : logits->rows, num_classes, std::max(ctx->count, 1),
                 training ? 1 : 0, ctx->xent_partials, s.get());
}

void BCEWithLogitsLoss::backward(const Stream &) const {}

}
```

parallel-gcn_amd/csrc/host/module.hpp:

```cpp
#pragma once
#include <memory>
#include <vector>

#include "comm.hpp"
#include "graph.hpp"
#include "runtime.hpp"

namespace pgcn {

using std::shared_ptr;

class Variable {
 public:
  DeviceBuffer<float> dev_data, dev_grad;
  DeviceBuffer<float> dev_grad_z;
  const Variable *skip_from = nullptr;
  int rows = 0, cols = 0, ld = 0;
  long long size = 0;
  Variable(int rows_, int cols_, bool requires_grad, int ld_ = -1);
  Variable() = default;
  void zero(hipStream_t s) const { dev_data.zero_async(s); }
  void zero_grad(hipStream_t s) const {
    if (dev_grad) dev_grad.zero_async(s);
  }
  std::vector<float> to_host(int which) const;
};

struct DevFeatures {
  bool dense = false;
  int rows = 0, cols = 0;
  long long nnz = 0;
  DeviceBuffer<float> x;
  int ldx = 0;
  DeviceBuffer<float> ax;
  DeviceBuffer<uint64_t> maskT;
  DeviceBuffer<uint64_t> maskW;
  DeviceBuffer<int> indptr, indices, csc_ptr, csc_row, csc_pos;
  DeviceBuffer<int> csc_order;
  DeviceBuffer<float> values;
  std::vector<float> host_values;
};

struct DropoutRng {
  DeviceBuffer<uint64_t> states;
  DeviceBuffer<uint64_t> mask;
  DeviceBuffer<uint64_t> mask_ahead;
  long long chunk_lo = 0, n_chunks = 0;
  int per = 2;
  long long elem_begin = 0, elem_end = 0;
  long long mask_base = 0;
};

class Module {
 public:
  virtual void forward(bool training, const Stream &s) const = 0;
  virtual void backward(const Stream &s) const = 0;
  virtual void set_num_samples(int) {}
  virtual int get_num_samples() const { return 0; }
  virtual ~Module() {}
};

class ReLU;
class GraphSum;
class Dropout;
class ResidualConnection;

struct ModuleContext {
  const Knobs *knobs = &process_knobs();
  bool train_ahead = true;
  hipStream_t side_stream = nullptr;
  hipStream_t tail_stream = nullptr;
  Event tail_fork, tail_done;
  bool tail_pending = false;
  bool tail_used = false;
  bool mm_side = false;
  Event mm_fork, side_join;
  void *gemm_workspace_side = nullptr;
  bool side_pending = false;
  DevGraph *split_graph = nullptr;
  const int *split_rows = nullptr;
  DevGraph *split_colgraph = nullptr;
  int compact_n = 0;
  const int *compact_truth = nullptr;
  Variable *compact_z = nullptr;
  Variable *compact_out = nullptr;
  const int *truth = nullptr;
  const uint32_t *label_bits = nullptr, *compact_label_bits = nullptr;
  int label_words = 0;
  int count = 0;
  float *xent_partials = nullptr;
  int xent_blocks = 0;
  const XentFinal *fin = nullptr;
  bool fin_taken = false;
  Comm *comm = nullptr;
  hipStream_t comm_stream = nullptr;
  int local_rows = 0;
  std::vector<DevGraph *> chunk_graphs;
  std::vector<DevGraph *> chunk_split_graphs;
  std::vector<const int *> chunk_split_rows;
  std::vector<DevGraph *> chunk_col_graphs;
  const void *jump_table = nullptr;
  XsDraw xs_draw;
  MaskDraw xs_draw_md[2];
  void *gemm_workspace = nullptr;
  size_t gemm_workspace_bytes = 0;
  bool profile = false;
  std::vector<std::pair<Event, Event>> *gs_events = nullptr;
  std::vector<double> *gs_bytes = nullptr;
  std::vector<std::pair<Event, Event>> *mm_events = nullptr;
  std::vector<double> *mm_flops = nullptr;
  std::vector<Event> *event_pool = nullptr;
};

void build_dev_features(DevFeatures &feats, const int *fptr, const int *indices,
                        const float *values, int first, int rows, int F, bool dense, int hidden0);
void init_dropout_rng_range(DropoutRng &r, const uint64_t seed[2], unsigned long long offset,
                            long long elem_begin, long long elem_end, int mask_per);
void glorot_fill(std::vector<float> &w, int in_size, int out_size, uint64_t s[2]);

class Dropout : public Module {
  shared_ptr<Variable> in;
  shared_ptr<DropoutRng> rng;
  float p;
  ModuleContext *ctx;

 public:
  Dropout(shared_ptr<Variable> in_, float p_, shared_ptr<DropoutRng> rng_, ModuleContext *ctx_);
  void forward(bool training, const Stream &s) const override;
  void backward(const Stream &s) const override;
  float scale() const { return 1.0f / (1.0f - p); }
  const DropoutRng &state() const { return *rng; }
  void draw_ahead(hipStream_t s, const Event *ready = nullptr) const;
  int ahead_descs(MaskDraw out[2]) const;
  bool drawn_ahead() const { return ahead; }
  void wait_ahead(hipStream_t s) const;
  const uint64_t *mask_ahead() const { return rng->mask_ahead.get(); }
  const Variable *variable() const { return in.get(); }
  void draw_fused(hipStream_t s) const;
  mutable bool skip_forward = false, skip_backward = false;
  const Dropout *co_draw = nullptr;
  mutable bool pre_drawn = false;
  void forget_draws() const {
    ahead = false;
    ahead_ready = nullptr;
    pre_drawn = false;
  }

 private:
  void draw(hipStream_t s, uint64_t *mask, int max_blocks = 0) const;
  mutable bool ahead = false;
  mutable const Event *ahead_ready = nullptr;
};

class SparseMatmul : public Module {
  const DevFeatures *x;
  shared_ptr<Variable> b, c;
  const Dropout *drop;
  ModuleContext *ctx;
  mutable bool last_training = false;
  mutable DeviceBuffer<float> ahead;
  mutable bool ahead_valid = false;

 public:
  SparseMatmul(const DevFeatures *x_, shared_ptr<Variable> b_, shared_ptr<Variable> c_,
               const Dropout *drop_, ModuleContext *ctx_);
  shared_ptr<Variable> eval_out;
  const GraphSum *consumer = nullptr;
  void forward(bool training, const Stream &s) const override;
  void backward(const Stream &s) const override;
  void forget_ahead() const { ahead_valid = false; }
};

class GraphSum : public Module {
  shared_ptr<Variable> in, out;
  DevGraph *graph;
  int dim;
  ModuleContext *ctx;
  bool last_layer;
 public:
  bool first_layer = false;
 private:
  mutable DeviceBuffer<float> compact;
  std::vector<DeviceBuffer<float>> partial;
  std::vector<Event> computed;
  Event reduced;

 public:
  GraphSum(shared_ptr<Variable> in_, shared_ptr<Variable> out_, DevGraph *graph_, int dim_,
           ModuleContext *ctx_, bool last_layer_ = false);
  void forward(bool training, const Stream &s) const override;
  void backward(const Stream &s) const override;
  const Variable *input() const { return in.get(); }
  const Variable *output() const { return out.get(); }
  int width() const { return dim; }
  ReLU *fwd_relu = nullptr;
  const ResidualConnection *fwd_res = nullptr;
  const Dropout *fwd_drop = nullptr;
  ReLU *bwd_relu = nullptr;
  const Dropout *bwd_drop = nullptr;
  GraphSum *fwd_next = nullptr, *bwd_next = nullptr;
  mutable bool prestaged_fwd = false, prestaged_bwd = false;
  DevGraph *forward_graph() const;
  DevGraph *backward_graph() const;
  DevGraph *forward_table_graph() const;
  DevGraph *backward_table_graph() const;
  float4 *claim_forward_table(int rows, int ld, const float **scale) const;
  bool claim_backward_table(int rows, int ld, XentTable *t) const;

 private:
  void run(const float *src, float *dst, const Stream &s, int mode = 0,
           const GsEpilogue *epi = nullptr, bool prestaged = false) const;
  void stage_next(GsEpilogue &e, GraphSum *next, DevGraph *ng, bool fwd) const;
  bool tail_ok(const DevGraph *g, int ld_in, int ld_out) const;
  GsEpilogue forward_epilogue(bool training, const Stream &s, const DevGraph *g) const;
  GsEpilogue backward_epilogue(const DevGraph *g) const;
  float *backward_dst(const GsEpilogue &e) const;
};

class GraphAttention : public Module {
  shared_ptr<Variable> in, out, attn;
  DevGraph *graph;
  int dim;
  long long offset;
  int heads;
  float p;
  shared_ptr<DropoutRng> rng;
  ModuleContext *ctx;
  DeviceBuffer<float> u, v, alpha, ws, z;

 public:
  static constexpr float kSlope = 0.2f;
  GraphAttention(shared_ptr<Variable> in_, shared_ptr<Variable> out_, DevGraph *graph_, int dim_,
                 shared_ptr<Variable> attn_, long long offset_, int heads_ = 1, float p_ = 0.0f,
                 shared_ptr<DropoutRng> rng_ = nullptr, ModuleContext *ctx_ = nullptr);
  void forward(bool training, const Stream &s) const override;
  void backward(const Stream &s) const override;
  const Variable *input() const { return in.get(); }
  const Variable *output() const { return out.get(); }
  int width() const { return dim; }
  int head_count() const { return heads; }
  const DropoutRng *mask_state() const { return rng.get(); }
  float scale() const { return 1.0f / (1.0f - p); }
};

class SageAggregate : public Module {
  shared_ptr<Variable> in, out;
  DevGraph *graph, *mean_fwd, *mean_bwd;
  int dim, aggregator;
  bool root;
  DeviceBuffer<int> arg;
  DeviceBuffer<float> q, dq;
  int ld_s;
  bool staged() const { return root && dim % 4 != 0; }

 public:
  SageAggregate(shared_ptr<Variable> in_, shared_ptr<Variable> out_, DevGraph *graph_,
                DevGraph *mean_fwd_, DevGraph *mean_bwd_, int dim_, int aggregator_, bool root_);
  void forward(bool training, const Stream &s) const override;
  void backward(const Stream &s) const override;
};

class Readout : public Module {
  shared_ptr<Variable> in, out;
  int n, G, dim, mode, max_len = 0;
  DeviceBuffer<int> graph_ptr, node_graph, arg;
  DeviceBuffer<float> ws;
  int ld_s;

 public:
  Readout(shared_ptr<Variable> in_, shared_ptr<Variable> out_, const std::vector<int> &graph_ptr_,
          int dim_, int mode_);
  const Variable *input() const { return in.get(); }
  const Variable *output() const { return out.get(); }
  int graphs() const { return G; }
  void forward(bool training, const Stream &s) const override;
  void backward(const Stream &s) const override;
};

class LinkDecoder : public Module {
  shared_ptr<Variable> in, out;
  const LinkIndexDev *links;
  int dim;

 public:
// ... 114 lines not shown
```

parallel-gcn_amd/csrc/k_elementwise.hip:

```cpp
#include <numeric>

#include "common.hpp"
#include "kernels.hpp"
#include "mask_draw.hpp"
#include "peer_sync.hpp"
#include "softmax_parts.hpp"

#pragma clang fp contract(off)

namespace pgcn {

__global__ __launch_bounds__(256) void k_dropout_mask(MaskSeg a, MaskSeg b, int blocks_a,
                                                      const uint4 *__restrict__ table) {
  __shared__ uint4 lut[32 * 16];
  for (int i = threadIdx.x; i < 32 * 16; i += blockDim.x) {
    const int p = i >> 4, v = i & 15;
    lut[i] = table[(p >> 1) * 256 + (v << (4 * (p & 1)))];
  }
  __syncthreads();
  const bool in_a = (int)blockIdx.x < blocks_a;
  const MaskSeg &sg = in_a ? a : b;
  const long long bid = in_a ? blockIdx.x : blockIdx.x - blocks_a;
  const long long nblk = in_a ? blocks_a : gridDim.x - blocks_a;
  if (sg.per == 2)
    dropout_mask_seg<2>(sg, lut, bid * blockDim.x + threadIdx.x, nblk * blockDim.x);
  else
    dropout_mask_seg<1>(sg, lut, bid * blockDim.x + threadIdx.x, nblk * blockDim.x);
}

__device__ __forceinline__ uint32_t mask_bits4(const uint64_t *__restrict__ mask, long long idx) {
  const long long w = idx >> 6;
  const int sh = (int)(idx & 63);
  uint64_t v = mask[w] >> sh;
  if (sh > 60) v |= mask[w + 1] << (64 - sh);
  return (uint32_t)v & 0xfu;
}

__global__ __launch_bounds__(256) void k_dropout_apply(float *__restrict__ x, long long n,
                                                       const uint64_t *__restrict__ mask,
                                                       long long base, float scale) {
  const long long n4 = n >> 2;
  for (long long q = (long long)blockIdx.x * blockDim.x + threadIdx.x; q < n4;
       q += (long long)gridDim.x * blockDim.x) {
    const long long i = q << 2;
    const uint32_t bits = mask_bits4(mask, base + i);
    float4 v = reinterpret_cast<float4 *>(x)[q];
    v.x *= (bits & 1) ? scale : 0.0f;
    v.y *= (bits & 2) ? scale : 0.0f;
    v.z *= (bits & 4) ? scale : 0.0f;
    v.w *= (bits & 8) ? scale : 0.0f;
    reinterpret_cast<float4 *>(x)[q] = v;
  }
  if (blockIdx.x == 0) {
    for (long long i = (n4 << 2) + threadIdx.x; i < n; i += blockDim.x) {
      const long long b = base + i;
      x[i] *= ((mask[b >> 6] >> (b & 63)) & 1) ? scale : 0.0f;
    }
  }
}

__global__ __launch_bounds__(256) void k_scatter_rows(const float4 *__restrict__ src,
                                                      const int *__restrict__ rows, int n, int ld4,
                                                      float4 *__restrict__ out) {
  const long long t = (long long)blockIdx.x * blockDim.x + threadIdx.x;
  if (t >= (long long)n * ld4) return;
  const long long r = t / ld4;
  const int q = (int)(t - r * ld4);
  out[(long long)rows[r] * ld4 + q] = src[t];
}

void launch_scatter_rows(const float *src, const int *rows, int n, int ld, float *out,
                         hipStream_t s) {
  PGCN_CHECK(ld % 4 == 0, PGCN_E_INVALID, "scatter_rows: ld % 4");
  if (n <= 0) return;
  const long long tot = (long long)n * (ld / 4);
  PGCN_LAUNCH(k_scatter_rows, dim3((unsigned)ceil_div(tot, 256)), dim3(256), 0, s,
                     reinterpret_cast<const float4 *>(src), rows, n, ld / 4,
                     reinterpret_cast<float4 *>(out));
}

__global__ __launch_bounds__(256) void k_gather_rows(const float4 *__restrict__ src,
                                                     const int *__restrict__ rows, int n, int ld4,
                                                     float4 *__restrict__ out) {
  const long long t = (long long)blockIdx.x * blockDim.x + threadIdx.x;
  if (t >= (long long)n * ld4) return;
  const long long r = t / ld4;
// ... 127 lines not shown
      gq += __uint_as_float(v.z);
    }
    gl = block_sum<XT>(gl, fred);
    gw = block_sum<XT>(gw, fred);
    gq = block_sum<XT>(gq, fred);
    const __amdgpu_buffer_rsrc_t gs = __builtin_amdgcn_make_buffer_rsrc(
        fin.gpart4, 0, (int)(n_top * 16), 0x00020000);
    if (threadIdx.x == 0) {
      const u4 d = {__float_as_uint(gl), __float_as_uint(gw), __float_as_uint(gq), 0u};
      __builtin_amdgcn_raw_buffer_store_b128(d, gs, (int)(g * 16), 0, 16);
      asm volatile("s_waitcnt vmcnt(0)" ::: "memory");
      __hip_atomic_store(fin.gticket + 16 * g, 0u, __ATOMIC_RELAXED, __HIP_MEMORY_SCOPE_AGENT);
      const unsigned old =
          __hip_atomic_fetch_add(fin.ticket, 1u, __ATOMIC_RELAXED, __HIP_MEMORY_SCOPE_AGENT);
      last = old == n_top - 1;
    }
    __syncthreads();
    if (!last) return;
  }
  float l = 0.0f, wr = 0.0f, w2 = 0.0f;
  {
    const __amdgpu_buffer_rsrc_t ts =
        G > 0 ? __builtin_amdgcn_make_buffer_rsrc(fin.gpart4, 0, (int)(n_top * 16), 0x00020000) : rs;
    for (int b = threadIdx.x; b < (int)n_top; b += blockDim.x) {
      const u4 v = __builtin_amdgcn_raw_buffer_load_b128(ts, b * 16, 0, 16);
      l += __uint_as_float(v.x);
      wr += __uint_as_float(v.y);
      w2 += __uint_as_float(v.z);
    }
  }
  l = block_sum<XT>(l, fred);
  wr = block_sum<XT>(wr, fred);
  w2 = block_sum<XT>(w2, fred);
  if (threadIdx.x == 0) {
    if (fin.sums) {
      fin.sums[0] = l;
      fin.sums[1] = wr;
    }
    float *o = fin.out2;
    if (fin.ctr) o += 4 * (fin.ctr[1] % fin.ring_cap);
    o[0] = l / (float)count + fin.wd * w2 / 2.0f;
    o[1] = (float)(count - (int)wr) / (float)count;
    __hip_atomic_store(fin.ticket, 0u, __ATOMIC_RELAXED, __HIP_MEMORY_SCOPE_AGENT);
  }
}


__device__ __forceinline__ void wave_lds_fence() {
  __builtin_amdgcn_wave_barrier();
  asm volatile("" ::: "memory");
}

__global__ void k_exp_check(const float *__restrict__ x, long long n, float *__restrict__ mine,
                            float *__restrict__ lib) {
  const long long i = (long long)blockIdx.x * blockDim.x + threadIdx.x;
  if (i < n) {
    mine[i] = exp_nonpos(x[i]);
    lib[i] = expf(x[i]);
  }
}

__global__ void k_div_check(const float *__restrict__ a, const float *__restrict__ b, long long n,
                            float *__restrict__ q) {
  const long long i = (long long)blockIdx.x * blockDim.x + threadIdx.x;
  if (i < n) q[i] = div_rn(a[i], b[i], 1.0f / b[i]);
}

void launch_exp_check(const float *x, long long n, float *mine, float *lib, hipStream_t s) {
  if (n <= 0) return;
  PGCN_LAUNCH(k_exp_check, dim3((unsigned)ceil_div(n, 256)), dim3(256), 0, s, x, n, mine, lib);
}

void launch_div_check(const float *a, const float *b, long long n, float *q, hipStream_t s) {
  if (n <= 0) return;
  PGCN_LAUNCH(k_div_check, dim3((unsigned)ceil_div(n, 256)), dim3(256), 0, s, a, b, n, q);
}

#ifdef PGCN_XENT_STAMPS
__device__ unsigned long long g_xent_stamps[16384 * 12];
#define XST(k) (st[k] = __builtin_amdgcn_s_memtime())
#else
#define XST(k) ((void)0)
#endif
template <bool FUSED, int CC = 0, int LDC = 0, int KH = 0>
__device__ __forceinline__ void xent_tile(float *__restrict__ logits, int ld_rt,
                                                  float *__restrict__ grad,
                                                  const int *__restrict__ truth, int n, int c_rt,
                                                  int count, int training,
                                                  float *__restrict__ partials, int write_back,
                                                  const float *__restrict__ H, int ldh, int kh_rt,
                                                  const float *__restrict__ W, int ldw,
                                                  float *__restrict__ dH, int lddh,
                                                  float *__restrict__ dWp, const XentTable &tb,
                                                  const XentFinal &fin) {
  extern __shared__ float smem[];
  __shared__ float red[2 * (XT / 64)];
#ifdef PGCN_XENT_STAMPS
  unsigned long long st[12] = {};
  st[10] = __builtin_amdgcn_s_memrealtime();
#endif
  const int c = CC > 0 ? CC : c_rt, ld = LDC > 0 ? LDC : ld_rt, kh = KH > 0 ? KH : kh_rt;
  XST(0);
  const int S = xent_stride(ld);
  const int wv = threadIdx.x >> 6, ln = threadIdx.x & 63, gi = ln >> 4, ii = ln & 15;
  const long long row0 = (long long)blockIdx.x * XR, wrow0 = row0 + 16 * wv;
  const int rows = (int)min((long long)XR, (long long)n - row0);
  const int wrows = max(0, min(16, rows - 16 * wv));
  float *L = smem + wv * 16 * S;
  const int ld4 = ld >> 2, tile4 = (wrows * ld) >> 2;
  const unsigned magic = (1u << 20) / (unsigned)ld4 + 1u;
  const long long base = wrow0 * ld;
  auto to_lds = [&](const float *src) {
    floatx4e v[8];
#pragma unroll
    for (int u = 0; u < 8; u++) {
      const int q = ln + 64 * u;
      if (q < tile4) v[u] = reinterpret_cast<const floatx4e *>(src + base)[q];
    }
#pragma unroll
    for (int u = 0; u < 8; u++) {
      const int q = ln + 64 * u;
      if (q < tile4) {
        const int r = (int)(__umul24((unsigned)q, magic) >> 20), j = 4 * (q - r * ld4);
        *reinterpret_cast<floatx4e *>(L + r * S + j) = v[u];
      }
    }
  };
  auto from_lds = [&](float *dst) {
    for (int q = ln; q < tile4; q += 64) {
      const int r = (int)(__umul24((unsigned)q, magic) >> 20), j = 4 * (q - r * ld4);
      reinterpret_cast<float4 *>(dst + base)[q] = *reinterpret_cast<const float4 *>(L + r * S + j);
    }
  };
  float *wt = smem + XR * S;
  float ha[4], hw[4];
  const int rq = ln >> 2, q = ln & 3;
  const int t = rq < wrows ? truth[wrow0 + rq] : -1;
  int tb_p = -1;
  float tb_s = 0.0f;
  if (FUSED && tb.table) {
    const int rr = 4 * gi + (ii & 3);
    const long long row = wrow0 + rr;
    tb_p = rr >= wrows ? -1 : (tb.pos ? tb.pos[row] : (row < tb.rows ? (int)row : -1));
  }
  if constexpr (FUSED) {
    const long long grow = wrow0 + ii < n ? wrow0 + ii : n - 1;
    const float *hr = H + grow * (long long)ldh;
    if (4 * gi + 3 < kh && ldh % 4 == 0) {
      const float4 h4 = *reinterpret_cast<const float4 *>(hr + 4 * gi);
      ha[0] = h4.x;
      ha[1] = h4.y;
      ha[2] = h4.z;
      ha[3] = h4.w;
    } else {
#pragma unroll
      for (int t4 = 0; t4 < 4; t4++) ha[t4] = 4 * gi + t4 < kh ? hr[4 * gi + t4] : 0.0f;
    }
    if (training && dWp) {
#pragma unroll
      for (int st = 0; st < 4; st++) {
        const int rloc = 4 * st + gi;
        hw[st] = (rloc < wrows && ii < kh) ? H[(wrow0 + rloc) * (long long)ldh + ii] : 0.0f;
      }
    }
    for (int k = wv; k < 16; k += XT / 64)
      for (int j = ln; j < ld; j += 64) wt[k * ld + j] = (k < kh && j < c) ? W[(long long)k * ldw + j] : 0.0f;
    __syncthreads();
    if (tb_p >= 0) tb_s = tb.scale[tb_p];
    XST(1);
    for (int tt = 0; 16 * tt < ld; tt++) {
      const int col = 16 * tt + ii;
      floatx4e acc = {0.f, 0.f, 0.f, 0.f};
#pragma unroll
      for (int t4 = 0; t4 < 4; t4++)
        acc = __builtin_amdgcn_mfma_f32_16x16x4f32(
            ha[t4], col < ld ? wt[(4 * gi + t4) * ld + col] : 0.0f, acc, 0, 0, 0);
      if (col < ld) {
#pragma unroll
        for (int r = 0; r < 4; r++) L[(4 * gi + r) * S + col] = acc[r];
      }
    }
  } else {
    to_lds(logits);
  }
  wave_lds_fence();
  XST(2);
  float loss = 0.0f, wrong = 0.0f, se = 0.0f;
  float *l = L + rq * S;
  constexpr int NV = 12;
  const bool regs = c <= 4 * NV;
  float v[NV];
  if (regs) {
#pragma unroll
    for (int k = 0; k < NV; k++) v[k] = q + 4 * k < c ? l[q + 4 * k] : -1e30f;
  }
  if (t >= 0) {
    float mx = -1e30f;
    if (regs) {
#pragma unroll
      for (int k = 0; k < NV; k++) mx = fmaxf(mx, v[k]);
    } else {
      for (int j = q; j < c; j += 4) mx = fmaxf(mx, l[j]);
    }
    mx = fmaxf(mx, __shfl_xor(mx, 1, 64));
    mx = fmaxf(mx, __shfl_xor(mx, 2, 64));
    bool w = false;
    float lt, s = 0.0f;
    if (regs) {
#pragma unroll
      for (int k = 0; k < NV; k++) {
        if (q + 4 * k < c) {
          v[k] -= mx;
          l[q + 4 * k] = v[k];
        }
      }
      wave_lds_fence();
      lt = l[t];
#pragma unroll
      for (int k = 0; k < NV; k++) w |= q + 4 * k < c && v[k] > lt;
#pragma unroll
      for (int k = 0; k < NV; k++) {
        if (q + 4 * k < c) {
          v[k] = exp_nonpos(v[k]);
          s += v[k];
        }
      }
    } else {
      for (int j = q; j < c; j += 4) {
        const float x = l[j] - mx;
        l[j] = x;
        s += exp_nonpos(x);
      }
      wave_lds_fence();
      lt = l[t];
      for (int j = q; j < c; j += 4) w |= l[j] > lt;
    }
    s += __shfl_xor(s, 1, 64);
    se = s + __shfl_xor(s, 2, 64);
    const int wq = (int)w | __shfl_xor((int)w, 1, 64);
    const int wall = wq | __shfl_xor(wq, 2, 64);
    if (q == 0) {
      loss = logf(se) - lt;
      wrong = wall ? 1.0f : 0.0f;
    }
  }
  wave_lds_fence();
  XST(3);
  if (write_back || FUSED) from_lds(logits);
  XST(4);
// ... 58 lines not shown
        if (p >= 0)
          reinterpret_cast<float4 *>(tb.table)[(long long)(p / RING_SR) * (4 * RING_SR) +
                                               v * RING_SR + p % RING_SR] =
              make_float4(o[0] * tb_s, o[1] * tb_s, o[2] * tb_s, o[3] * tb_s);
      }
    }
    XST(6);
    if (FUSED && dWp) {
      floatx4e pw[3] = {{0.f, 0.f, 0.f, 0.f}, {0.f, 0.f, 0.f, 0.f}, {0.f, 0.f, 0.f, 0.f}};
#pragma unroll
      for (int st = 0; st < 4; st++) {
        const int rloc = 4 * st + gi;
        const bool ok = rloc < wrows;
#pragma unroll
        for (int tt = 0; tt < 3; tt++) {
          const int col = 16 * tt + ii;
          const float bv = (ok && col < ld) ? L[rloc * S + col] : 0.0f;
          pw[tt] = __builtin_amdgcn_mfma_f32_16x16x4f32(hw[st], bv, pw[tt], 0, 0, 0);
        }
      }
      from_lds(grad);
      XST(7);
      wave_lds_fence();
#pragma unroll
      for (int tt = 0; tt < 3; tt++)
#pragma unroll
        for (int r = 0; r < 4; r++) L[(tt * 4 + r) * 64 + ln] = pw[tt][r];
      __syncthreads();
      if (wv == 0) {
        float *pb = dWp + (long long)blockIdx.x * kh * 48;
#pragma unroll
        for (int tt = 0; tt < 3; tt++)
#pragma unroll
          for (int r = 0; r < 4; r++) {
            float v = pw[tt][r];
#pragma unroll
            for (int w2 = 1; w2 < XT / 64; w2++) v += smem[w2 * 16 * S + (tt * 4 + r) * 64 + ln];
            if (4 * gi + r < kh) pb[(4 * gi + r) * 48 + 16 * tt + ii] = v;
          }
      }
    } else {
      from_lds(grad);
    }
  }
  XST(8);
  loss = wave_sum(loss);
  wrong = wave_sum(wrong);
  if (ln == 0) {
    red[2 * wv] = loss;
    red[2 * wv + 1] = wrong;
  }
  __syncthreads();
  if (threadIdx.x == 0) {
    float ls = red[0], ws = red[1];
#pragma unroll
    for (int w2 = 1; w2 < XT / 64; w2++) {
      ls += red[2 * w2];
      ws += red[2 * w2 + 1];
    }
    partials[2 * blockIdx.x] = ls;
    partials[2 * blockIdx.x + 1] = ws;
    red[0] = ls;
    red[1] = ws;
  }
  if (fin.ticket) xent_finish(fin, count, red);
  XST(9);
#ifdef PGCN_XENT_STAMPS
  st[11] = __builtin_amdgcn_s_memrealtime();
  const long long wslot = (long long)blockIdx.x * (XT / 64) + wv;
  if (ln < 12 && wslot < 16384) {
    unsigned long long x = st[0];
#pragma unroll
    for (int k = 1; k < 12; k++) x = ln == k ? st[k] : x;
    g_xent_stamps[wslot * 12 + ln] = x;
  }
#endif
}

#define PGCN_XENT_ARGS                                                                          \
  float *__restrict__ logits, int ld, float *__restrict__ grad, const int *__restrict__ truth,   \
      int n, int c, int count, int training, float *__restrict__ partials, int write_back,       \
      const float *__restrict__ H, int ldh, int kh, const float *__restrict__ W, int ldw,        \
      float *__restrict__ dH, int lddh, float *__restrict__ dWp, XentTable tb, XentFinal fin
__global__ __launch_bounds__(XT) void k_xent_fwd(PGCN_XENT_ARGS) {
  xent_tile<false>(logits, ld, grad, truth, n, c, count, training, partials, write_back, H, ldh,
                   kh, W, ldw, dH, lddh, dWp, tb, fin);
}
template <int CC, int LDC, int KH>
__global__ __launch_bounds__(XT) __attribute__((amdgpu_waves_per_eu(8))) void k_out_xent(
    PGCN_XENT_ARGS) {
  xent_tile<true, CC, LDC, KH>(logits, ld, grad, truth, n, c, count, training, partials,
                               write_back, H, ldh, kh, W, ldw, dH, lddh, dWp, tb, fin);
}
#undef PGCN_XENT_ARGS

__global__ __launch_bounds__(1024) void k_reduce_scalars(const float *__restrict__ partials,
                                                         int n_blocks,
                                                         const float *__restrict__ w,
                                                         long long n_w, float *__restrict__ sums,
                                                         int count, float wd,
                                                         float *__restrict__ out2,
                                                         const int *__restrict__ ctr,
                                                         int ring_cap, float *__restrict__ raw4,
                                                         PeerSmall peer) {
  __shared__ float red[16];
  float l = 0.0f, wr = 0.0f, q = 0.0f;
  constexpr int U = 8;
  for (int b0 = threadIdx.x; b0 < n_blocks; b0 += U * 1024) {
    float2 v[U];
#pragma unroll
    for (int u = 0; u < U; u++)
      if (b0 + u * 1024 < n_blocks) v[u] = reinterpret_cast<const float2 *>(partials)[b0 + u * 1024];
#pragma unroll
    for (int u = 0; u < U; u++)
      if (b0 + u * 1024 < n_blocks) {
        l += v[u].x;
        wr += v[u].y;
      }
  }
  constexpr int UW = 32;
  for (long long i0 = threadIdx.x; i0 < n_w; i0 += UW * 1024) {
    float v[UW];
#pragma unroll
    for (int u = 0; u < UW; u++) v[u] = i0 + u * 1024 < n_w ? w[i0 + u * 1024] : 0.0f;
#pragma unroll
    for (int u = 0; u < UW; u++)
      if (i0 + u * 1024 < n_w) q += v[u] * v[u];
  }
  l = block_sum<1024>(l, red);
  wr = block_sum<1024>(wr, red);
  q = block_sum<1024>(q, red);
  if (threadIdx.x == 0) {
    if (sums) {
      sums[0] = l;
      sums[1] = wr;
    }
    if (raw4) {
      raw4[0] = l;
      raw4[1] = wr;
      raw4[2] = q;
      raw4[3] = (float)count;
    }
    if (out2) {
      if (ctr) out2 += 4 * (ctr[1] % ring_cap);
      out2[0] = l / (float)count + wd * q / 2.0f;
      out2[1] = (float)(count - (int)wr) / (float)count;
    }
  }
  if (raw4 && peer.k.world) {
    __syncthreads();
    (void)peer_allreduce_block(raw4, 2, peer);
  }
}

__device__ __forceinline__ void adam_range(float *__restrict__ w, const float *__restrict__ g,
                                           float *__restrict__ m, float *__restrict__ v,
                                           long long n, float step_size, float beta1,
                                           float beta2, float eps, float wd, int decay,
                                           const TnDeferred &red = TnDeferred{},
                                           const PeerRecv *peer = nullptr, long long off = 0,
                                           long long bid = -1, long long nblk = 0) {
  const double ob1 = 1.0 - (double)beta1, ob2 = 1.0 - (double)beta2;
  if (bid < 0) {
    bid = blockIdx.x;
    nblk = gridDim.x;
  }
  for (long long i = bid * blockDim.x + threadIdx.x; i < n; i += nblk * blockDim.x) {
    float grad;
    if (peer) {
      float p[kPeerMaxRanks];
#pragma unroll
      for (int q = 0; q < kPeerMaxRanks; q++)
        if (q < peer->world) p[q] = peer->slot[q][off + i];
      grad = p[0];
#pragma unroll
      for (int q = 1; q < kPeerMaxRanks; q++)
// ... 124 lines not shown
  for (int i = 0; i < 2; i++) {
    sg[i].states = d[i]->states;
    sg[i].n_chunks = d[i]->n_chunks;
    sg[i].elem0 = d[i]->elem0;
    sg[i].elem_end = d[i]->elem_end;
    sg[i].threshold = (int)(d[i]->p * (float)0x7fffffff);
    sg[i].mask = d[i]->mask;
    PGCN_CHECK(d[i]->per == 1 || d[i]->per == 2, PGCN_E_INVALID, "dropout_mask2: words per state");
    sg[i].per = d[i]->per;
    g[i] = sg[i].n_chunks > 0 ? grid_for(ceil_div(ceil_div(sg[i].n_chunks, d[i]->per), 2), 256,
                                         8 * kCUs)
                              : 0;
  }
  if (g[0] + g[1] == 0) return;
  PGCN_LAUNCH(k_dropout_mask, dim3(g[0] + g[1]), dim3(256), 0, s, sg[0], sg[1], g[0],
              static_cast<const uint4 *>(table));
}

void launch_dropout_apply_based(float *x, long long n, const uint64_t *mask, long long base,
                                float scale, hipStream_t s) {
  if (n <= 0) return;
  PGCN_LAUNCH(k_dropout_apply, dim3(grid_for(ceil_div(n, 4))), dim3(256), 0, s, x, n,
                     mask, base, scale);
}

void launch_relu_fwd(float *x, long long n, uint8_t *mask, int training, hipStream_t s) {
  if (n <= 0) return;
  PGCN_LAUNCH(k_relu_fwd, dim3(grid_for(n)), dim3(256), 0, s, x, n, mask, training);
}

void launch_relu_bwd(float *g, long long n, const uint8_t *mask, hipStream_t s) {
  if (n <= 0) return;
  PGCN_LAUNCH(k_relu_bwd, dim3(grid_for(n)), dim3(256), 0, s, g, n, mask);
}

void launch_relu_bwd_to(const float *g, long long n, const uint8_t *mask, float *z,
                        hipStream_t s) {
  if (n <= 0) return;
  PGCN_LAUNCH(k_relu_bwd_to, dim3(grid_for(n)), dim3(256), 0, s, g, n, mask, z);
}

static void launch_add_into(float *y, const float *x, long long n, hipStream_t s) {
  if (n <= 0) return;
  const bool al = ((reinterpret_cast<uintptr_t>(y) | reinterpret_cast<uintptr_t>(x)) & 15) == 0;
  const long long n4 = al ? n / 4 : 0;
  PGCN_LAUNCH(k_add_into, dim3(grid_for(std::max(n4, n - 4 * n4))), dim3(256), 0, s, y, x, n4, n);
}

void launch_residual_fwd(float *cur, const float *prev, long long n, hipStream_t s) {
  launch_add_into(cur, prev, n, s);
}

void launch_residual_bwd(float *prev_grad, const float *cur_grad, long long n, hipStream_t s) {
  launch_add_into(prev_grad, cur_grad, n, s);
}

int xent_blocks(int n) { return (int)ceil_div(n, XR); }

__global__ void k_empty() {}

void launch_empty(int n, hipStream_t s) {
  for (int i = 0; i < n; i++) hipLaunchKernelGGL(k_empty, dim3(1), dim3(64), 0, s);
}

void launch_xent_fwd(float *logits, int ld, float *grad, const int *truth, int n, int c,
                     int count, int training, float *partials, hipStream_t s, int write_back,
                     const XentFinal *fin) {
  if (n <= 0) return;
  PGCN_CHECK(ld <= 124 && c <= ld && ld % 4 == 0, PGCN_E_INVALID,
             "xent: classes must be <= 124 (ld a multiple of 4)");
  PGCN_CHECK(!fin || (fin->ticket && fin->part4 && fin->out2 &&
                      (fin->group == 0 || (fin->group > 0 && fin->gticket && fin->gpart4))),
             PGCN_E_INVALID,
             "xent: the fused finish needs its ticket, partials and output");
  const size_t lds = (size_t)XR * xent_stride(ld) * sizeof(float);
  PGCN_LAUNCH(k_xent_fwd, dim3(xent_blocks(n)), dim3(XT), lds, s, logits, ld, grad,
                     truth, n, c, count, training, partials, write_back, nullptr, 0, 0, nullptr, 0,
                     nullptr, 0, nullptr, XentTable{}, fin ? *fin : XentFinal{});
}

void launch_out_xent(const float *H, int ldh, int kh, const float *W, int ldw, float *logits,
                     int ld, float *grad, const int *truth, int n, int c, int count, int training,
                     float *partials, hipStream_t s, float *dH, int lddh, float *dWp,
                     const XentTable *tb, const XentFinal *fin) {
  note_path(KP_OUT_XENT);
  PGCN_CHECK(!fin || (fin->ticket && fin->part4 && fin->out2 &&
                      (fin->group == 0 || (fin->group > 0 && fin->gticket && fin->gpart4))),
             PGCN_E_INVALID,
             "out_xent: the fused finish needs its ticket, partials and output");
  const XentTable t = training && dH && tb ? *tb : XentTable{};
  PGCN_CHECK(!t.table || (kh == 16 && t.scale), PGCN_E_INVALID,
             "out_xent: a prescaled table of a 16-column dH");
  if (n <= 0) return;
  PGCN_CHECK(ld <= 116 && c <= ld && ld % 4 == 0 && kh >= 1 && kh <= 16, PGCN_E_INVALID,
             "out_xent: classes <= 116, hidden <= 16");
  PGCN_CHECK(!dWp || ld <= 48, PGCN_E_INVALID, "out_xent: the weight-grad partial needs <= 48 classes");
  const size_t lds = ((size_t)XR * xent_stride(ld) + (size_t)16 * ld) * sizeof(float);
#define OUT_XENT(...)                                                                          \
  PGCN_LAUNCH((k_out_xent<__VA_ARGS__>), dim3(xent_blocks(n)), dim3(XT), lds, s, logits, ld, grad, \
              truth, n, c, count, training, partials, 1, H, ldh, kh, W, ldw,                     \
              training ? dH : nullptr, lddh, training ? dWp : nullptr, t, fin ? *fin : XentFinal{})
  if (c == 41 && ld == 44 && kh == 16)
    OUT_XENT(41, 44, 16);
  else if (c == 7 && ld == 8 && kh == 16)
    OUT_XENT(7, 8, 16);
  else if (c == 6 && ld == 8 && kh == 16)
    OUT_XENT(6, 8, 16);
  else if (c == 3 && ld == 4 && kh == 16)
    OUT_XENT(3, 4, 16);
  else
    OUT_XENT(0, 0, 0);
#undef OUT_XENT
}

void launch_reduce_scalars(const float *partials, int n_blocks, const float *w, long long n_w,
                           float *sums, hipStream_t s, int count, float wd, float *out2,
                           const int *ctr, int ring_cap, float *raw4, const PeerSmall *peer) {
  PGCN_CHECK(!peer || (raw4 && peer->k.world >= 1 && peer->k.world <= kPeerMaxRanks),
             PGCN_E_INVALID, "reduce_scalars: peer all-reduce of the raw pair");
  PGCN_LAUNCH(k_reduce_scalars, dim3(1), dim3(1024), 0, s, partials, n_blocks, w, n_w,
                     sums, count, wd, out2, ctr, ring_cap, raw4, peer ? *peer : PeerSmall{});
}

__global__ void k_counters(int *ctr, int set, int step, int epoch) {
  if (threadIdx.x == 0) {
    if (set) {
      ctr[0] = step;
      ctr[1] = epoch;
    } else {
      ctr[0] += 1;
      ctr[1] += 1;
    }
  }
}

void launch_counters(int *ctr, int set, int step, int epoch, hipStream_t s) {
  PGCN_LAUNCH(k_counters, dim3(1), dim3(64), 0, s, ctr, set, step, epoch);
}

void launch_adam_multi(const AdamBatch &b, float step_size, float beta1, float beta2, float eps,
                       float wd, hipStream_t s, const float *step_table, const int *ctr,
                       int table_cap, const MaskDraw *draws, int n_draws, const void *table) {
  if (b.count <= 0) return;
  long long nmax = 0;
  for (int t = 0; t < b.count; t++) nmax = std::max(nmax, b.n[t]);
  if (n_draws > 0) {
    PGCN_CHECK(!step_table && !b.peer.world && n_draws <= 2 && table, PGCN_E_INVALID,
               "adam_mask: eager one-GPU steps, at most two masks, the jump table");
    MaskSeg sg[2];
    int g[2] = {0, 0};
    for (int i = 0; i < n_draws; i++) {
      const MaskDraw &d = draws[i];
      PGCN_CHECK(d.per == 1 || d.per == 2, PGCN_E_INVALID, "adam_mask: words per state");
      sg[i].states = d.states;
      sg[i].n_chunks = d.n_chunks;
      sg[i].elem0 = d.elem0;
      sg[i].elem_end = d.elem_end;
      sg[i].threshold = (int)(d.p * (float)0x7fffffff);
      sg[i].mask = d.mask;
      sg[i].per = d.per;
      g[i] = d.n_chunks > 0 ? grid_for(ceil_div(ceil_div(d.n_chunks, d.per), 2), 256, 8 * kCUs) : 0;
    }
    const int ga = grid_for(nmax);
    PGCN_LAUNCH(k_adam_mask, dim3((unsigned)(g[0] + g[1] + ga * b.count)), dim3(256), 0, s, b,
                step_size, beta1, beta2, eps, wd, sg[0], sg[1], g[0], g[1], ga,
                static_cast<const uint4 *>(table));
    return;
  }
  PGCN_LAUNCH(k_adam_multi, dim3(grid_for(nmax), b.count), dim3(256), 0, s, b, step_size,
                     beta1, beta2, eps, wd, step_table, ctr, table_cap);
}

void launch_adam(float *w, const float *g, float *m, float *v, long long n, float step_size,
                 float beta1, float beta2, float eps, float wd, int decay, hipStream_t s,
                 const float *step_table, const int *ctr, int table_cap) {
  if (n <= 0) return;
  PGCN_LAUNCH(k_adam, dim3(grid_for(n)), dim3(256), 0, s, w, g, m, v, n, step_size,
                     beta1, beta2, eps, wd, decay, step_table, ctr, table_cap);
}

#ifdef PGCN_XENT_STAMPS
extern "C" int pgcn_debug_xent_stamps(unsigned long long *host, long long n) {
  if (n > 16384LL * 12) n = 16384LL * 12;
  return hipMemcpyFromSymbol(host, HIP_SYMBOL(g_xent_stamps), (size_t)n * 8, 0,
                             hipMemcpyDeviceToHost) == hipSuccess ? 0 : -1;
// ... 4 lines not shown
```

parallel-gcn_amd/csrc/k_graphsum_ring.hip:

```cpp
#include "common.hpp"
#include "gs_epilogue.hpp"
#include "kernels.hpp"
#include "lds_dma.hpp"
#include "peer_sync.hpp"

namespace pgcn {

constexpr int RING_PLANE_B = RING_P * 16;
constexpr int RING_TABLE_B = 4 * RING_PLANE_B;
constexpr int RING_CNT_USED = LDS_CW * LDS_SLOTS * 2;
constexpr int RING_CNT_B = 512;
constexpr int RING_NCB_MAX = RING_K - 1;
constexpr int RING_CNT_OFF = RING_TABLE_B;
constexpr int RING_FLAG_OFF = RING_CNT_OFF + RING_CNT_USED;
constexpr int RING_NFLAGS = 1 + RING_K;
constexpr int RING_ERING_OFF = RING_CNT_OFF + RING_NCB_MAX * RING_CNT_B;
constexpr int RING_CHUNK = 512;
constexpr int RING_ESLOTS = 4;
constexpr int RING_ERING_B = RING_ESLOTS * RING_CHUNK;
constexpr int RING_TOTAL_B = RING_ERING_OFF + LDS_CW * RING_ERING_B;
static_assert(RING_TOTAL_B <= 160 * 1024, "LDS budget");
static_assert(RING_FLAG_OFF + RING_NFLAGS * 4 <= RING_CNT_OFF + RING_CNT_B,
              "hand-off words fit");
static_assert(RING_SR * 16 % 1024 == 0, "a slice's plane piece is whole 1-KB LDS-DMA pieces");
// ... 333 lines not shown
      unsigned long long saved;
      const unsigned daddr = lds_base + (unsigned)(RING_FLAG_OFF + 4 * (1 + t % RING_K));
      asm volatile(
          "s_mov_b64 %1, exec\n\t"
          "s_mov_b64 exec, 1\n\t"
          "ds_add_rtn_u32 %0, %2, %3\n\t"
          "s_waitcnt lgkmcnt(0)\n\t"
          "s_mov_b64 exec, %1"
          : "=&v"(rank), "=&s"(saved)
          : "v"(daddr), "v"(1u)
          : "memory");
    }
    rank = (unsigned)__builtin_amdgcn_readfirstlane((int)rank) - (unsigned)(LDS_CW * (t / RING_K));
    if (rank >= (unsigned)(2 * LDS_CW / 3)) __builtin_amdgcn_s_setprio(2);
    else if (rank >= (unsigned)(LDS_CW / 3)) __builtin_amdgcn_s_setprio(1);
    else __builtin_amdgcn_s_setprio(0);
  }
  asm volatile("s_waitcnt vmcnt(0)" ::: "memory");
  const int *rw = rows + (((long long)batch * LDS_CW + wave) * NS) * 16 + g;
  float4 *pb = partial + (long long)b * part_stride * 4 + v;
  int uw[NS];
#pragma unroll
  for (int j = 0; j < NS; j++) uw[j] = rw[j * 16];
#pragma unroll
  for (int j = 0; j < NS; j++) {
    const int u = uw[j];
    const int sp = __builtin_amdgcn_readfirstlane((int)((unsigned)u >> 28));
    float4 a = make_float4(acc[j].x, acc[j].y, acc[j].z, acc[j].w);
    for (int k = 0; k < sp; k++) {
      const int d = 4 << k;
      a.x += __shfl_xor(a.x, d);
      a.y += __shfl_xor(a.y, d);
      a.z += __shfl_xor(a.z, d);
      a.w += __shfl_xor(a.w, d);
    }
    const int r = u & kRingRowMask;
    if (r != kRingEmpty && (g & ((1 << sp) - 1)) == 0) pb[(long long)r * 4] = a;
  }
}


void launch_gs_finish(float *y, int ld, int n, int dim, const GsEpilogue &epi, hipStream_t st) {
  PGCN_CHECK(ld % 4 == 0 && dim % 4 == 0 && dim <= ld && n >= 0, PGCN_E_INVALID,
             "gs_finish: shape");
  PGCN_CHECK(!epi.next_table || dim == 16, PGCN_E_INVALID, "gs_finish: next table of a wide row");
  if (n == 0 || epi.mode == 0) return;
  const long long t = (long long)n * (dim / 4);
  PGCN_LAUNCH(k_gs_finish, dim3((unsigned)ceil_div(t, 256)), dim3(256), 0, st,
              reinterpret_cast<float4 *>(y), ld / 4, n, dim / 4, epi);
  PGCN_HIP(hipGetLastError());
}

void launch_gs_gather_finish(float *y, int ld, int n, int dim, const GsEpilogue &epi,
                             const PeerRecv &r, hipStream_t st) {
  PGCN_CHECK(ld % 4 == 0 && dim % 4 == 0 && dim <= ld && n >= 0 && r.world >= 1 &&
                 r.world <= kPeerMaxRanks,
             PGCN_E_INVALID, "gs_gather_finish: shape");
  PGCN_CHECK(!epi.next_table || dim == 16, PGCN_E_INVALID,
             "gs_gather_finish: next table of a wide row");
  if (n == 0) return;
  const long long t = (long long)n * (dim / 4);
  PGCN_LAUNCH(k_gs_gather_finish, dim3((unsigned)ceil_div(t, 256)), dim3(256), 0, st,
              reinterpret_cast<float4 *>(y), ld / 4, n, dim / 4, epi, r);
  PGCN_HIP(hipGetLastError());
}

void launch_ring_prescale_wide(const LdsSchedule &s, const float *in, int ld_in, int width,
                               const RingPasses &passes, float *tables, long long table_floats,
                               hipStream_t st) {
  PGCN_CHECK(ld_in % 4 == 0 && width % 4 == 0 && width <= 128 && passes.n >= 1 && passes.n <= 8,
             PGCN_E_INVALID, "ring_prescale_wide: shape");
  for (int p = 0; p < passes.n; p++)
    PGCN_CHECK(passes.c[p] % 4 == 0 && passes.c[p] + 16 <= width, PGCN_E_INVALID,
               "ring_prescale_wide: pass columns");
  PGCN_LAUNCH(k_ring_prescale_wide, dim3((unsigned)ceil_div(s.n_cols, RPW_ROWS)), dim3(256), 0, st,
              in, ld_in, width, s.col_scale, s.n_cols, passes, reinterpret_cast<float4 *>(tables),
              table_floats / 4);
  PGCN_HIP(hipGetLastError());
}

void launch_graphsum_ring(const LdsSchedule &s, const float *in, int ld_in, float *out,
                          int ld_out, float *scratch_in, float *partial, hipStream_t st,
                          const int *col_map, const GsEpilogue *epi, bool prestaged,
                          const PeerSink *push, hipStream_t tail_st, hipEvent_t fork) {
  note_path(KP_GS_RING);
  PGCN_CHECK(!tail_st || (push && fork), PGCN_E_INVALID, "graphsum_ring: tail stream of a push");
  PGCN_CHECK(ld_in % 4 == 0 && ld_out % 4 == 0, PGCN_E_INVALID, "graphsum_ring: ld % 4");
  const long long pre = (long long)s.n_cols * 4;
  if (!prestaged)
    PGCN_LAUNCH(k_ring_prescale, dim3((unsigned)ceil_div(pre, 256)), dim3(256), 0, st,
                       reinterpret_cast<const float4 *>(in), ld_in / 4, s.col_scale, s.n_cols,
                       reinterpret_cast<float4 *>(scratch_in), col_map);
  const long long n_wg = (long long)s.n_batches * s.n_blocks;
#define RING_LAUNCH(NS_, PAIR_, WIN_)                                                           \
  PGCN_LAUNCH((k_graphsum_ring<NS_, PAIR_, WIN_>), dim3((unsigned)n_wg), dim3(LDS_THREADS), 0, st, s.entries, \
              s.wave_off, s.counts, s.t_max, s.slices, s.n_slices, s.rows,                      \
              reinterpret_cast<const char *>(scratch_in), reinterpret_cast<float4 *>(partial), \
              (long long)s.n_rows, s.n_blocks)
  PGCN_CHECK(ring_slots_ok(s.ns), PGCN_E_INVALID, "graphsum_ring: rowsets per wave");
  PGCN_CHECK((s.w == 2 || s.w == 3) && (!s.pair || s.w == 3), PGCN_E_INVALID,
             "graphsum_ring: window (pairs: 3 only)");
  if (s.pair)
    RING_LAUNCH(16, true, 3);
  else if (s.w == 2)
    RING_LAUNCH(16, false, 2);
  else
    RING_LAUNCH(16, false, 3);
#undef RING_LAUNCH
  const GsEpilogue none{};
  const long long post = (long long)s.n_rows * 4;
  if (push) {
    PGCN_CHECK((!epi || epi->mode == 0) && push->world >= 1 && push->world <= kPeerMaxRanks &&
                   push->rows_per_rank > 0 && (long long)push->rows_per_rank * push->world >= s.n_rows,
               PGCN_E_INVALID, "graphsum_ring: push shape");
    const long long tiles = (long long)push->world * ceil_div(push->rows_per_rank, 64);
    const long long blocks = std::min<long long>(ceil_div(tiles, 4), (long long)kCUs);
    if (tail_st) {
      PGCN_HIP(hipEventRecord(fork, st));
      PGCN_HIP(hipStreamWaitEvent(tail_st, fork, 0));
      st = tail_st;
    }
    PGCN_LAUNCH(k_gs_lds_combine<true>, dim3((unsigned)blocks), dim3(1024), 0, st,
                reinterpret_cast<const float4 *>(partial), (long long)s.n_rows, s.n_blocks,
                s.row_scale, s.n_rows, nullptr, ld_out / 4, none, *push);
  } else {
    PGCN_LAUNCH(k_gs_lds_combine<false>, dim3((unsigned)ceil_div(post, 256)), dim3(256), 0, st,
                reinterpret_cast<const float4 *>(partial), (long long)s.n_rows, s.n_blocks,
                s.row_scale, s.n_rows, reinterpret_cast<float4 *>(out), ld_out / 4,
                epi ? *epi : none, PeerSink{});
  }
  PGCN_HIP(hipGetLastError());
}

}
```

parallel-gcn_amd/csrc/kernels.hpp:

```cpp
#pragma once
#include <hip/hip_runtime.h>

#include <cstddef>
#include <cstdint>

#include "gs_epilogue.hpp"

namespace pgcn {

enum KernelPath {
  KP_XS_NN_RING, KP_XS_TN_RING, KP_XS_NN, KP_XS_TN, KP_GS_RING, KP_GS_GATHER, KP_OUT_XENT,
  KP_GEMM_NN, KP_GEMM_TN, KP_GEMM_NN_W, KP_GEMM_TN_W, KP_GAT_FWD, KP_GAT_BWD, KP_GAT_HEADS,
  KP_SPMM_CSR, KP_SPMM_CSR_DUAL, KP_SPMM_CSC_256, KP_SPMM_CSC_1024, KP_SPMM_TREE_256,
  KP_SPMM_TREE_1024, KP_LAUNCHES, KP_LINK_FWD, KP_LINK_BWD, KP_COUNT
};
void note_path(KernelPath p);
#define PGCN_LAUNCH(...)                     \
  do {                                       \
    ::pgcn::note_path(::pgcn::KP_LAUNCHES);  \
    hipLaunchKernelGGL(__VA_ARGS__);         \
  } while (0)
void launch_empty(int n, hipStream_t s);
void launch_exp_check(const float *x, long long n, float *mine, float *lib, hipStream_t s);
void launch_div_check(const float *a, const float *b, long long n, float *q, hipStream_t s);

struct GraphSchedule {
  int vec = 0;
  int chunk = 0;
  int nbc = 1;
  int n_items = 0;
  int max_block_items = 0;
  int n_comb = 0;
  long long n_slots = 0;
  const int4 *items = nullptr;
  const int *block_items = nullptr;
  const int4 *comb = nullptr;
  const int *slot_comb = nullptr;
  int *comb_ctr = nullptr;
  int n_wide = 0;
  const int4 *wide = nullptr;
  int gather16 = 0;
};
int graphsum_group_lanes(int vec);

void launch_graphsum(const GraphSchedule &s, const int *indices, const float *vals,
                     const float *in, int ld_in, float *out, int ld_out, float *partial,
                     hipStream_t st, const GsEpilogue *epi = nullptr);
bool graphsum_vec_supported(int vec);

constexpr int kGraphBlocks = 8;
constexpr int LDS_CW = 15;
constexpr int LDS_SLOTS = 16;
constexpr bool ring_slots_ok(int ns) { return ns == LDS_SLOTS; }
constexpr int LDS_THREADS = 64 * (LDS_CW + 1);
#ifndef PGCN_RING_SR
#define PGCN_RING_SR 512
#endif
#ifndef PGCN_RING_K
#define PGCN_RING_K 4
#endif
#ifndef PGCN_RING_W
#define PGCN_RING_W (PGCN_RING_K - 1)
#endif
constexpr int RING_SR = PGCN_RING_SR;
constexpr int RING_K = PGCN_RING_K;
constexpr int RING_W = PGCN_RING_W;
static_assert(RING_W >= 1 && RING_W <= RING_K - 1 && RING_SR % 64 == 0, "ring shape");
constexpr int RING_P = RING_K * RING_SR + 4;
constexpr int kRingWindow = 5;
constexpr int kRingRowMask = 0x0fffffff;
constexpr int kRingEmpty = 0x0fffffff;
static_assert(RING_P % 16 == 4, "plane stride: lane v's chunk = 4v + row (mod 16)");
struct LdsSchedule {
  int n_rows = 0, n_cols = 0;
  int n_batches = 0;
  int n_blocks = 4;
  int t_max = 0;
  int ns = LDS_SLOTS;
  bool pair = false;
  int w = RING_W;
  const uint2 *entries = nullptr;
  const long long *wave_off = nullptr;
  const unsigned short *counts = nullptr;
  const int2 *slices = nullptr;
  const int *n_slices = nullptr;
  const int *rows = nullptr;
  const float *row_scale = nullptr;
  const float *col_scale = nullptr;
};
struct RingPasses {
  int n = 0;
  int c[8] = {0, 0, 0, 0, 0, 0, 0, 0};
};
void launch_ring_prescale_wide(const LdsSchedule &s, const float *in, int ld_in, int width,
                               const RingPasses &passes, float *tables, long long table_floats,
                               hipStream_t st);
void launch_graphsum_ring(const LdsSchedule &s, const float *in, int ld_in, float *out,
                          int ld_out, float *scratch_in, float *partial, hipStream_t st,
                          const int *col_map = nullptr, const GsEpilogue *epi = nullptr,
                          bool prestaged = false, const struct PeerSink *push = nullptr,
                          hipStream_t tail_st = nullptr, hipEvent_t fork = nullptr);
void launch_gs_finish(float *y, int ld, int n, int dim, const GsEpilogue &epi, hipStream_t st);

void launch_gemm_nn(int M, int N, int K, const float *A, int lda, const float *B, int ldb,
                    int trans_b, float *C, int ldc, const uint64_t *a_mask, long long mask_base,
                    long long mask_ld, float a_scale, hipStream_t s,
                    const uint64_t *maskT = nullptr);
size_t gemm_tn_workspace(int M, int N, int K);
bool gemm_wide_ok(int N);
void launch_gemm_nn_wide(int M, int N, int K, const float *A, int lda, const float *B, int ldb,
                         int trans_b, float *C, int ldc, const uint64_t *a_mask,
                         long long mask_base, long long mask_ld, float a_scale, hipStream_t s,
                         int nst, const uint64_t *maskT = nullptr);
size_t gemm_tn_wide_workspace(int M, int N, int K);
void launch_gemm_tn_wide(int M, int N, int K, const float *A, int lda, const float *G, int ldg,
                         float *C, int ldc, const uint64_t *a_mask, long long mask_base,
                         long long mask_ld, float a_scale, void *workspace, hipStream_t s,
                         int nst, const uint64_t *maskT = nullptr);
void launch_slab_reduce(float *partial, int n_slabs, int K, int N, int ldp, float *C, int ldc,
                        int nst, hipStream_t s);
bool xstream_ok(int N, int K);
void launch_mask_nibbles(const uint64_t *mask, long long mask_base, long long mask_ld, int M,
                         int K, uint64_t *out, hipStream_t s);
struct MaskSeg {
  uint64_t *states = nullptr;
  long long n_chunks = 0, elem0 = 0, elem_end = 0;
  int threshold = 0;
  uint64_t *mask = nullptr;
  int per = 1;
};
struct XsDraw {
  MaskSeg seg[2];
  int n = 0;
  const uint4 *lut = nullptr;
};
struct XsEpilogue {
  int relu = 0;
  const uint64_t *bwd_drop = nullptr;
  long long drop_base = 0;
  float drop_scale = 0.0f;
  const uint8_t *bwd_relu = nullptr;
  float4 *next_table = nullptr;
  const float *next_scale = nullptr;
  int next_sr = 0;
  const XsDraw *draw = nullptr;
};
struct XsMask {
  const uint64_t *bits = nullptr;
  long long base = 0, ld = 0;
  long long words = 0;
};
void launch_xstream_nn(int M, int N, int K, const float *A, int lda, const float *B, int ldb,
                       int trans_b, float *C, int ldc, const uint64_t *maskT, float a_scale,
                       hipStream_t s, float *C2 = nullptr,
                       const XsEpilogue *epi = nullptr, const XsMask *flat = nullptr);
bool xstream_ring_ok(int K, int lda);
void launch_xstream_nn_ring(int M, int N, int K, const float *A, int lda, const float *B, int ldb,
                            int trans_b, float *C, int ldc, const uint64_t *maskT, float a_scale,
                            hipStream_t s, float *C2, const XsEpilogue &e,
                            const XsMask *flat = nullptr);
void launch_xstream_tn_ring(int M, int N, int K, const float *A, int lda, const float *G, int ldg,
                            const uint64_t *maskT, float a_scale, float *partial, int n_blocks,
                            hipStream_t s, const XsMask *flat = nullptr);
void launch_gather_rows(const float *src, const int *rows, int n, int ld, float *out,
                        hipStream_t s);
constexpr int kPeerMaxRanks = 16;
constexpr unsigned long long kPeerTimeoutTicks = 2000000000ull;
struct PeerSink {
  float *dst[kPeerMaxRanks];
  unsigned *flag[kPeerMaxRanks];
  unsigned *arrive = nullptr;
  long long slot_bytes = 0;
  unsigned gen = 0;
  int world = 0;
  int rows_per_rank = 0;
  int signal = 1;
  const unsigned *wait_flags = nullptr;
  int nwait = 0;
  unsigned *err = nullptr;
};
struct PeerRecv {
  const float *slot[kPeerMaxRanks];
  int world = 0;
};
// ... 74 lines not shown
  int n = 0;
  long long nnz = 0;
  const int *indptr = nullptr, *indices = nullptr;
  const int *csc_ptr = nullptr, *csc_row = nullptr, *csc_pos = nullptr;
  int n_row_segs = 0, n_col_segs = 0, n_long_cols = 0;
  const int4 *row_segs = nullptr, *col_segs = nullptr;
  const int2 *long_cols = nullptr;
  float *row_ws = nullptr;
};
bool gat_heads_ok(int d, int heads);
void launch_gat_scores(const float *P, int ld_p, int n, int d, int heads, const float *a_dst,
                       const float *a_src, float *u, float *v, hipStream_t s);
void launch_gat_fwd(const GatPattern &g, const float *P, int ld_p, const float *u, const float *v,
                    float slope, float *Z, int ld_z, int d, int heads, const uint64_t *drop_mask,
                    long long drop_base, float drop_scale, float *alpha, hipStream_t s);
size_t gat_bwd_workspace(const GatPattern &g, int d, int heads);
void launch_gat_bwd(const GatPattern &g, const float *P, int ld_p, const float *u, const float *v,
                    float slope, const float *alpha, const float *Z, int ld_z, const float *G,
                    int ld_g, const float *a_dst, const float *a_src, float *dP, int ld_dp, int d,
                    int heads, const uint64_t *drop_mask, long long drop_base, float drop_scale,
                    float *da, void *workspace, hipStream_t s);
constexpr int kSageMaxWidth = kGatMaxWidth;
constexpr int kSageWsStride = kSageMaxWidth;
struct SageWs {
  float *row_val = nullptr;
  int *row_arg = nullptr;
  float *col_ws = nullptr;
};
void launch_agg_max_fwd(const GatPattern &g, const SageWs &ws, const float *in, int ld_in, int d,
                        const float *add, int ld_add, float *out, int ld_out, int *arg,
                        int ld_arg, hipStream_t s);
void launch_agg_max_bwd(const GatPattern &g, const SageWs &ws, const float *G, int ld_g,
                        const int *arg, int ld_arg, int d, float *din, int ld_din, hipStream_t s);
void launch_copy_cols(const float *src, int ld_src, float *dst, int ld_dst, int n, int cols,
                      bool add, hipStream_t s);
constexpr int kReadoutChunk = 512;
constexpr int kReadoutMaxWidth = kSageMaxWidth;
constexpr int kReadoutWsStride = kReadoutMaxWidth;
enum { kReadoutNone = 0, kReadoutSum = 1, kReadoutMean = 2, kReadoutMax = 3 };
size_t readout_workspace(int n);
void launch_readout_fwd(const float *in, int ld_in, const int *graph_ptr, int G, int n, int d,
                        int mode, int max_len, float *out, int ld_out, int *arg, int ld_arg,
                        void *workspace, hipStream_t s);
void launch_readout_bwd(const float *Gout, int ld_g, const int *graph_ptr, const int *node_graph,
                        const int *arg, int ld_arg, int G, int n, int d, int mode, float *din,
                        int ld_din, hipStream_t s);
constexpr int kLinkMaxWidth = kSageMaxWidth;
constexpr int kLinkWsStride = kLinkMaxWidth;
struct LinkIndex {
  int n = 0;
  long long n_pairs = 0;
  const int *src = nullptr, *dst = nullptr;
  const int *inc_ptr = nullptr, *inc_pair = nullptr, *inc_other = nullptr;
  int n_segs = 0, n_long = 0;
  const int4 *segs = nullptr;
  const int2 *longs = nullptr;
  float *ws = nullptr;
};
void launch_link_score_fwd(const LinkIndex &l, const float *H, int ld_h, int d, float *scores,
                           int ld_s, hipStream_t s);
void launch_link_score_bwd(const LinkIndex &l, const float *H, int ld_h, int d, const float *G,
                           int ld_g, float *dH, int ld_dh, hipStream_t s);
int xent_blocks(int n);
struct XentTable {
  float *table = nullptr;
  const float *scale = nullptr;
  const int *pos = nullptr;
  int rows = 0;
};
struct XentFinal {
  const float *w = nullptr;
  long long n_w = 0;
  float wd = 0.0f;
  float *out2 = nullptr;
  const int *ctr = nullptr;
  int ring_cap = 1;
  float *sums = nullptr;
  unsigned *ticket = nullptr;
  float4 *part4 = nullptr;
  int group = 0;
  unsigned *gticket = nullptr;
  float4 *gpart4 = nullptr;
};
void launch_out_xent(const float *H, int ldh, int kh, const float *W, int ldw, float *logits,
                     int ld, float *grad, const int *truth, int n, int c, int count, int training,
                     float *partials, hipStream_t s, float *dH = nullptr, int lddh = 0,
                     float *dWp = nullptr, const XentTable *tb = nullptr,
                     const XentFinal *fin = nullptr);
void launch_tn_reduce_blocks(float *partial, int n_blocks, int K, int N, int ldp, float *C, int ldc,
                             hipStream_t s);
float *tn_defer_blocks(int n_blocks, int K, int N, int ldp, float *C, int ldc);
void launch_tn_reduce_one_pass(const float *partial, int n, int K, int N, int ldp, float *C,
                               int ldc, hipStream_t s);
size_t tn_reduce_blocks_workspace(int n_blocks, int K, int ldp);
void launch_xent_fwd(float *logits, int ld, float *grad, const int *truth, int n, int c,
                     int count, int training, float *partials, hipStream_t s, int write_back = 1,
                     const XentFinal *fin = nullptr);
constexpr int kPredictRows = 64, kPredictMaxClasses = 128;
void launch_predict_rows(const float *logits, int ld, int n, int c, int *cls, float *conf,
                         float *probs, int ld_probs, hipStream_t s);
void launch_confusion(const int *cls, const int *truth, int n, int c, unsigned int *counts,
                      hipStream_t s);
void check_bce_args(int ld, int words, int n, int c, int count);
void launch_bce_fwd(const float *logits, int ld, float *grad, const int *truth,
                    const uint32_t *label_bits, int words, int n, int c, int count, int training,
                    float *partials, hipStream_t s);
void check_predict_multilabel_args(int ld, int n, int c, int words, bool probs, int ld_probs);
void launch_predict_multilabel(const float *logits, int ld, int n, int c, uint32_t *bits,
                               int words, float *probs, int ld_probs, hipStream_t s);
void check_multilabel_counts_args(int n, int c, int words);
void launch_multilabel_counts(const uint32_t *pred_bits, const uint32_t *label_bits,
                              const int *truth, int n, int c, int words, unsigned int *counts,
                              hipStream_t s);
void launch_reduce_scalars(const float *partials, int n_blocks, const float *w, long long n_w,
                           float *sums, hipStream_t s, int count = 0, float wd = 0.0f,
                           float *out2 = nullptr, const int *ctr = nullptr, int ring_cap = 1,
                           float *raw4 = nullptr, const PeerSmall *peer = nullptr);
void launch_adam(float *w, const float *g, float *m, float *v, long long n, float step_size,
                 float beta1, float beta2, float eps, float wd, int decay, hipStream_t s,
                 const float *step_table = nullptr, const int *ctr = nullptr, int table_cap = 1);
constexpr int kAdamBatch = 8;
struct TnDeferred {
  const float *src = nullptr;
  int n_groups = 0, K = 0, N = 0, ldp = 0;
  float *C = nullptr;
};
struct TnDeferList {
  int n = 0;
  TnDeferred d[4];
  float *pool = nullptr;
  size_t pool_floats = 0, used = 0;
};
void tn_defer(TnDeferList *list);
void tn_defer_flush(TnDeferList &list, hipStream_t s);

struct AdamBatch {
  float *w[kAdamBatch];
  const float *g[kAdamBatch];
  float *m[kAdamBatch], *v[kAdamBatch];
  long long n[kAdamBatch];
  int decay[kAdamBatch];
  int count;
  TnDeferred red[kAdamBatch];
  PeerRecv peer;
  long long arena_off[kAdamBatch];
};
struct GradRegions {
  int n = 0;
  long long off[4];
  TnDeferred d[4];
};
void launch_peer_push_grads(const float *arena, long long n, const GradRegions &r,
                            const PeerSink &k, hipStream_t s);
void launch_adam_multi(const AdamBatch &b, float step_size, float beta1, float beta2, float eps,
                       float wd, hipStream_t s, const float *step_table = nullptr,
                       const int *ctr = nullptr, int table_cap = 1,
                       const MaskDraw *draws = nullptr, int n_draws = 0,
                       const void *table = nullptr);
void launch_counters(int *ctr, int set, int step, int epoch, hipStream_t s);

}
```

parallel-gcn_amd/csrc/knobs.cpp:

```cpp
#include "knobs.hpp"

#include <algorithm>
#include <climits>
#include <cstring>

namespace pgcn {
static constexpr KnobScope E = KnobScope::Engine, G = KnobScope::Graph, P = KnobScope::Process;
#define PGCN_KNOB(field, scope, lo, hi) {#field, &Knobs::field, scope, lo, hi, 0, {}}
#define PGCN_KNOB_LIST(field, scope, n, ...) {#field, &Knobs::field, scope, 0, 0, n, {__VA_ARGS__}}
const KnobRow kKnobTable[] = {
    PGCN_KNOB(train_ahead, E, 0, 1),
    PGCN_KNOB(split_rows, E, 0, 1),
    PGCN_KNOB(split_cols, E, 0, 1),
    PGCN_KNOB(eval_ax, E, 0, 1),
    PGCN_KNOB(epoch_graph, E, 0, 1),
    PGCN_KNOB(fuse_epilogue, E, 0, 15),
    PGCN_KNOB(fuse_output, E, 0, 3),
    PGCN_KNOB(mm_side, E, 0, 2),
    PGCN_KNOB(eval_tail, E, 0, 1),
    PGCN_KNOB(co_draw, E, 0, 2),
    PGCN_KNOB(sparse_dual, E, 0, 1),
    PGCN_KNOB(tn_fold, E, 0, 1),
    PGCN_KNOB(fuse_finish, E, 0, 2),
    PGCN_KNOB(mask_per, E, 0, 2),
    PGCN_KNOB(csc_tree, E, 0, 1),
    PGCN_KNOB(mask_adam, E, 0, 1),
    PGCN_KNOB(mask_xstream, E, 0, 1),
    PGCN_KNOB(reassoc_small, E, 0, 1),
    PGCN_KNOB(defer_wgrad, E, 0, 1),
    PGCN_KNOB(peer_uncached, E, 0, 1),
    PGCN_KNOB(lds_min_kb, G, INT_MIN, INT_MAX),
    PGCN_KNOB_LIST(lds_blocks, G, 7, 0, 1, 2, 4, 8, 16, 32),
    PGCN_KNOB(gs_split, G, 0, 3),
    PGCN_KNOB_LIST(gs_item_iters, G, 6, 0, 2, 4, 8, 16, 32),
    PGCN_KNOB(gs_orig_cols, G, 0, 1),
    PGCN_KNOB(gs16_gather, G, 0, 2),
    PGCN_KNOB(ring_pair, G, 0, 1),
    PGCN_KNOB_LIST(ring_window, G, 3, 0, 2, 3),
    PGCN_KNOB(parse_threads, P, 0, 4096),
    PGCN_KNOB(xstream_ring, P, 0, 1),
};
#undef PGCN_KNOB
#undef PGCN_KNOB_LIST
const int kKnobCount = (int)(sizeof(kKnobTable) / sizeof(kKnobTable[0]));

bool KnobRow::accepts(int v) const {
  if (!n_allowed) return v >= lo && v <= hi;
  return std::find(allowed, allowed + n_allowed, v) != allowed + n_allowed;
}

const KnobRow *find_knob(const char *name) {
  for (int i = 0; i < kKnobCount; i++)
    if (!std::strcmp(kKnobTable[i].name, name)) return &kKnobTable[i];
  return nullptr;
}

Knobs &process_knobs() {
  static Knobs k;
  return k;
}

}
```

parallel-gcn_amd/csrc/knobs.hpp:

```cpp
#pragma once

namespace pgcn {

constexpr int kFuseTails = 1, kFusePrestage = 2, kFuseXstream = 4, kFuseMatmulTails = 8;

struct Knobs {
  int train_ahead = 1;
  int split_rows = 0;
  int split_cols = 1;
  int eval_ax = 1;
  int epoch_graph = 0;
  int fuse_epilogue = kFuseTails | kFusePrestage | kFuseXstream | kFuseMatmulTails;
  int fuse_output = 2;
  int mm_side = 0;
  int eval_tail = 0;
  int co_draw = 2;
  int sparse_dual = 1;
  int tn_fold = 1;
  int fuse_finish = 1;
  int mask_per = 0;
  int csc_tree = 0;
  int mask_adam = 1;
  int mask_xstream = 0;
  int reassoc_small = 1;
  int defer_wgrad = 1;
  int peer_uncached = 0;
  int lds_min_kb = -1;
  int lds_blocks = 0;
  int gs_split = 3;
  int gs_item_iters = 0;
  int gs_orig_cols = 1;
  int gs16_gather = 0;
  int ring_pair = 0;
  int ring_window = 0;
  int parse_threads = 0;
  int xstream_ring = 1;
};

enum class KnobScope { Engine, Graph, Process };
struct KnobRow {
  const char *name;
  int Knobs::*field;
  KnobScope scope;
  int lo, hi, n_allowed, allowed[7];
  bool accepts(int v) const;
};
extern const KnobRow kKnobTable[];
extern const int kKnobCount;
const KnobRow *find_knob(const char *name);
Knobs &process_knobs();

}
```

Measured before the change: 615.4.

## Fold GraphSum ring-partial combine into the fused output cross-entropy kernel

When the last GraphSum feeds the fused output matmul plus cross-entropy, the ring SpMM now stops after writing per-block partials. It skips its separate combine kernel and hands the partial descriptors to the loss. The out_xent kernel gets a partials variant that sums up to 8 block partials per row, applies the row scale, writes H back, and goes straight on to the logits. This removes one kernel launch and one full write-then-read pass over H. The cost is extra partial loads inside the xent kernel, more register pressure, and a cross-module handoff through shared context state.

```diff
diff --git a/include/pgcn.h b/include/pgcn.h
--- a/include/pgcn.h
+++ b/include/pgcn.h
@@ -333,6 +333,16 @@
                         int training, float *partials, float *dH, int lddh, float *dWp,
                         float *table, const float *scale, const int *pos, int table_rows,
                         const pgcn_xent_final *fin, void *stream);
+int pgcn_debug_out_xent_partials(const float *partial, long long part_stride, int n_blocks,
+                                 const float *scale_row, float *H, int ldh, const float *W,
+                                 int ldw, float *logits, int ld, float *grad, const int *truth,
+                                 int n, int c, int count, int training, float *partials,
+                                 float *dH, int lddh, float *dWp, float *table,
+                                 const float *scale, const int *pos, int table_rows,
+                                 const pgcn_xent_final *fin, void *stream);
+int pgcn_debug_ring_combine(const float *partial, long long part_stride, int n_blocks,
+                            const float *scale_row, int n, float *out, int ld_out, void *stream);
+int pgcn_debug_out_xent_fold(int on);
 int pgcn_debug_finalize_ring(const float *partials, int n_blocks, int count, const float *w_l2,
                              long long n_l2, float weight_decay, float *out2, const int *ctr,
                              int ring_cap, float *sums, void *stream);
diff --git a/parallel-gcn_amd/__init__.py b/parallel-gcn_amd/__init__.py
--- a/parallel-gcn_amd/__init__.py
+++ b/parallel-gcn_amd/__init__.py
@@ -236,6 +236,12 @@
 _sig("pgcn_debug_out_xent", c_int, c_void_p, c_int, c_int, c_void_p, c_int, c_void_p, c_int,
      c_void_p, c_void_p, c_int, c_int, c_int, c_int, c_void_p, c_void_p, c_int, c_void_p,
      c_void_p, c_void_p, c_void_p, c_int, P(PgcnXentFinal), c_void_p)
+_sig("pgcn_debug_out_xent_partials", c_int, c_void_p, c_ll, c_int, c_void_p, c_void_p, c_int,
+     c_void_p, c_int, c_void_p, c_int, c_void_p, c_void_p, c_int, c_int, c_int, c_int, c_void_p,
+     c_void_p, c_int, c_void_p, c_void_p, c_void_p, c_void_p, c_int, P(PgcnXentFinal), c_void_p)
+_sig("pgcn_debug_ring_combine", c_int, c_void_p, c_ll, c_int, c_void_p, c_int, c_void_p, c_int,
+     c_void_p)
+_sig("pgcn_debug_out_xent_fold", c_int, c_int)
 _sig("pgcn_debug_finalize_ring", c_int, c_void_p, c_int, c_int, c_void_p, c_ll, c_float,
      c_void_p, c_void_p, c_int, c_void_p, c_void_p)
 _sig("pgcn_debug_tn_reduce_blocks_workspace", c_size_t, c_int, c_int, c_int)
@@ -286,7 +292,8 @@
 KERNEL_PATHS = ("xs_nn_ring", "xs_tn_ring", "xs_nn", "xs_tn", "gs_ring", "gs_gather", "out_xent",
                 "gemm_nn", "gemm_tn", "gemm_nn_w", "gemm_tn_w", "gat_fwd", "gat_bwd", "gat_heads",
                 "spmm_csr", "spmm_csr_dual", "spmm_csc_256", "spmm_csc_1024", "spmm_tree_256",
-                "spmm_tree_1024", "launches", "link_fwd", "link_bwd")
+                "spmm_tree_1024", "launches", "link_fwd", "link_bwd", "gs_combine",
+                "out_xent_part")
 
 
 def path_counts(reset=False, thread=False):
@@ -984,6 +991,7 @@
     "pgcn_debug_lds_check", "pgcn_debug_lds_counts", "pgcn_debug_path_count",
     "pgcn_debug_empty_launches", "pgcn_debug_exp_check", "pgcn_debug_div_check",
     "pgcn_debug_ring_slice_rows", "pgcn_debug_xent_fwd", "pgcn_debug_out_xent",
+    "pgcn_debug_out_xent_partials", "pgcn_debug_ring_combine", "pgcn_debug_out_xent_fold",
     "pgcn_debug_finalize_ring", "pgcn_debug_tn_reduce_blocks_workspace",
     "pgcn_debug_tn_reduce_blocks", "pgcn_debug_tn_reduce_one_pass",
     "pgcn_debug_gemm_nib", "pgcn_debug_gemm_tn_nib",
diff --git a/parallel-gcn_amd/csrc/capi.cpp b/parallel-gcn_amd/csrc/capi.cpp
--- a/parallel-gcn_amd/csrc/capi.cpp
+++ b/parallel-gcn_amd/csrc/capi.cpp
@@ -28,7 +28,8 @@
                                           "gat_bwd",    "gat_heads",  "spmm_csr",
                                           "spmm_csr_dual", "spmm_csc_256", "spmm_csc_1024",
                                           "spmm_tree_256", "spmm_tree_1024", "launches",
-                                          "link_fwd",   "link_bwd"};
+                                          "link_fwd",   "link_bwd",   "gs_combine",
+                                          "out_xent_part"};
 }
 void note_path(KernelPath p) {
   g_path_hits[p].fetch_add(1, std::memory_order_relaxed);
@@ -1651,6 +1652,75 @@
   });
 }
 
+int pgcn_debug_out_xent_partials(const float *partial, long long part_stride, int n_blocks,
+                                 const float *scale_row, float *H, int ldh, const float *W,
+                                 int ldw, float *logits, int ld, float *grad, const int *truth,
+                                 int n, int c, int count, int training, float *partials,
+                                 float *dH, int lddh, float *dWp, float *table,
+                                 const float *scale, const int *pos, int table_rows,
+                                 const pgcn_xent_final *fin, void *stream) {
+  return guarded([&] {
+    PGCN_CHECK(n >= 0 && ldh >= 16 && ldh % 4 == 0 && n_blocks >= 1 &&
+                   n_blocks <= kXentMaxPartials && part_stride >= n,
+               PGCN_E_INVALID,
+               "debug_out_xent_partials: ldh >= 16, ldh % 4 == 0, 1 <= n_blocks <= 8, "
+               "part_stride >= n");
+    PGCN_CHECK(c >= 1 && c <= ld && ld <= 116 && ld % 4 == 0 && ldw >= c && count >= 0,
+               PGCN_E_INVALID,
+               "debug_out_xent_partials: 1 <= c <= ld <= 116, ld % 4 == 0, ldw >= c");
+    PGCN_CHECK(!dH || lddh >= 16, PGCN_E_INVALID, "debug_out_xent_partials: lddh >= 16");
+    PGCN_CHECK(!dWp || ld <= 48, PGCN_E_INVALID,
+               "debug_out_xent_partials: the weight-grad partial needs <= 48 classes");
+    PGCN_CHECK(!table || (scale && dH && (pos || table_rows >= 0)), PGCN_E_INVALID,
+               "debug_out_xent_partials: a prescaled table of dH");
+    PGCN_CHECK(n == 0 || (partial && scale_row && H && W && logits && truth && partials &&
+                          (grad || !training)),
+               PGCN_E_INVALID, "debug_out_xent_partials: null argument");
+    check_final(fin, "debug_out_xent_partials: the finish needs its ticket, partials and output");
+    if (n == 0) return;
+    XentFinal xf;
+    if (fin) xf = to_final(*fin);
+    XentTable tb;
+    tb.table = table;
+    tb.scale = scale;
+    tb.pos = pos;
+    tb.rows = table_rows;
+    RingPartials rp;
+    rp.partial = reinterpret_cast<const float4 *>(partial);
+    rp.part_stride = part_stride;
+    rp.n_blocks = n_blocks;
+    rp.row_scale = scale_row;
+    launch_out_xent(H, ldh, 16, W, ldw, logits, ld, grad, truth, n, c, count, training, partials,
+                    as_stream(stream), dH, lddh, dWp, table ? &tb : nullptr,
+                    fin ? &xf : nullptr, &rp);
+    PGCN_HIP(hipGetLastError());
+  });
+}
+
+int pgcn_debug_ring_combine(const float *partial, long long part_stride, int n_blocks,
+                            const float *scale_row, int n, float *out, int ld_out, void *stream) {
+  return guarded([&] {
+    PGCN_CHECK(n >= 0 && n_blocks >= 1 && part_stride >= n && ld_out >= 16 && ld_out % 4 == 0,
+               PGCN_E_INVALID,
+               "debug_ring_combine: n_blocks >= 1, part_stride >= n, ld_out >= 16, ld_out % 4 == 0");
+    PGCN_CHECK(n == 0 || (partial && scale_row && out), PGCN_E_INVALID,
+               "debug_ring_combine: null argument");
+    if (n == 0) return;
+    RingPartials rp;
+    rp.partial = reinterpret_cast<const float4 *>(partial);
+    rp.part_stride = part_stride;
+    rp.n_blocks = n_blocks;
+    rp.row_scale = scale_row;
+    launch_ring_combine(rp, n, out, ld_out, as_stream(stream));
+  });
+}
+
+int pgcn_debug_out_xent_fold(int on) {
+  if (on != 0 && on != 1) return PGCN_E_INVALID;
+  out_xent_fold() = on;
+  return PGCN_OK;
+}
+
 int pgcn_debug_finalize_ring(const float *partials, int n_blocks, int count, const float *w_l2,
                              long long n_l2, float weight_decay, float *out2, const int *ctr,
                              int ring_cap, float *sums, void *stream) {
diff --git a/parallel-gcn_amd/csrc/host/gcn.cpp b/parallel-gcn_amd/csrc/host/gcn.cpp
--- a/parallel-gcn_amd/csrc/host/gcn.cpp
+++ b/parallel-gcn_amd/csrc/host/gcn.cpp
@@ -811,7 +811,10 @@
   ce->fused = mm;
   mm->fused_forward = true;
   auto *gs = n >= 3 ? dynamic_cast<GraphSum *>(modules[n - 3].get()) : nullptr;
-  if (gs && gs->output() == mm->input()) ce->dh_reader = gs;
+  if (gs && gs->output() == mm->input()) {
+    ce->dh_reader = gs;
+    gs->feeds_out_xent = true;
+  }
 }
 
 void GCN::fuse_epilogues() {
diff --git a/parallel-gcn_amd/csrc/host/graph.cpp b/parallel-gcn_amd/csrc/host/graph.cpp
--- a/parallel-gcn_amd/csrc/host/graph.cpp
+++ b/parallel-gcn_amd/csrc/host/graph.cpp
@@ -595,6 +595,16 @@
                   epi);
 }
 
+bool DevGraph::graphsum_partials(const float *in, int ld_in, int dim, hipStream_t s,
+                                 bool prestaged, RingPartials *p) {
+  if (dim != 16 || ld_in % 4 != 0 || ld_in < 16 || !uses_lds(dim)) return false;
+  if (!lds_) build_lds();
+  if (lds_->s.n_blocks > kXentMaxPartials) return false;
+  launch_graphsum_ring(lds_->s, in, ld_in, nullptr, 16, table_scratch(), lds_->partial.get(), s,
+                       col_map_.get(), nullptr, prestaged, nullptr, nullptr, nullptr, p);
+  return true;
+}
+
 static void gat_segments(int n, const std::vector<int> &ptr, std::vector<int4> *segs,
                          std::vector<int2> *longs) {
   for (int i = 0; i < n; i++) {
diff --git a/parallel-gcn_amd/csrc/host/graph.hpp b/parallel-gcn_amd/csrc/host/graph.hpp
--- a/parallel-gcn_amd/csrc/host/graph.hpp
+++ b/parallel-gcn_amd/csrc/host/graph.hpp
@@ -58,6 +58,8 @@
                 bool compact_in = false, const GsEpilogue *epi = nullptr, bool prestaged = false,
                 bool tables_ready = false, const PeerSink *push = nullptr,
                 hipStream_t tail_st = nullptr, hipEvent_t fork = nullptr);
+  bool graphsum_partials(const float *in, int ld_in, int dim, hipStream_t s, bool prestaged,
+                         RingPartials *p);
   void share_tables(DevGraph *owner);
   bool can_share_tables(int dim, int ld_in) const;
   const DevGraph *table_owner() const { return table_owner_; }
diff --git a/parallel-gcn_amd/csrc/host/module.cpp b/parallel-gcn_amd/csrc/host/module.cpp
--- a/parallel-gcn_amd/csrc/host/module.cpp
+++ b/parallel-gcn_amd/csrc/host/module.cpp
@@ -546,6 +546,14 @@
   DevGraph *sg = last_layer && !ctx->comm ? ctx->split_graph : nullptr;
   if (!sg) {
     const GsEpilogue epi = forward_epilogue(training, s, graph);
+    if (feeds_out_xent && out_xent_fold() && !ctx->comm && !ctx->profile && !ctx->compact_n &&
+        epi.mode == 0 && !epi.next_table && dim == 16 && out->ld % 4 == 0 && out->ld >= 16 &&
+        graph->rows() == out->rows &&
+        graph->graphsum_partials(in->dev_data.get(), in->ld, dim, s.get(), pre,
+                                 &ctx->out_partials)) {
+      ctx->out_partials_of = out.get();
+      return;
+    }
     run(in->dev_data.get(), out->dev_data.get(), s, 0, &epi, pre);
     return;
   }
@@ -966,6 +974,10 @@
 
 
 void CrossEntropyLoss::forward(bool training, const Stream &s) const {
+  const Variable *part_of = ctx->out_partials_of;
+  ctx->out_partials_of = nullptr;
+  PGCN_CHECK(!part_of || (fused && !ctx->compact_n && part_of == fused->input()), PGCN_E_INVALID,
+             "loss: GraphSum partials handed to a loss that does not sum them");
   if (fused && !ctx->compact_n) {
     const Variable &Hv = *fused->input(), &Wv = *fused->weight();
     const double mm = 2.0 * logits->rows * num_classes * fused->inner();
@@ -997,7 +1009,8 @@
     launch_out_xent(Hv.dev_data.get(), Hv.ld, fused->inner(), Wv.dev_data.get(), Wv.ld,
                     logits->dev_data.get(), logits->ld, training ? logits->dev_grad.get() : nullptr,
                     ctx->truth, logits->rows, num_classes, ctx->count, training ? 1 : 0,
-                    ctx->xent_partials, s.get(), dH, Hv.ld, dWp, staged ? &tb : nullptr, ctx->fin);
+                    ctx->xent_partials, s.get(), dH, Hv.ld, dWp, staged ? &tb : nullptr, ctx->fin,
+                    part_of ? &ctx->out_partials : nullptr);
     ctx->fin_taken = ctx->fin != nullptr;
     if (one_pass)
       launch_tn_reduce_one_pass(dWp, nb, fused->inner(), num_classes, 48, Wv.dev_grad.get(),
diff --git a/parallel-gcn_amd/csrc/host/module.hpp b/parallel-gcn_amd/csrc/host/module.hpp
--- a/parallel-gcn_amd/csrc/host/module.hpp
+++ b/parallel-gcn_amd/csrc/host/module.hpp
@@ -92,6 +92,8 @@
   int xent_blocks = 0;
   const XentFinal *fin = nullptr;
   bool fin_taken = false;
+  RingPartials out_partials;
+  const Variable *out_partials_of = nullptr;
   Comm *comm = nullptr;
   hipStream_t comm_stream = nullptr;
   int local_rows = 0;
@@ -200,6 +202,7 @@
   const Dropout *bwd_drop = nullptr;
   GraphSum *fwd_next = nullptr, *bwd_next = nullptr;
   mutable bool prestaged_fwd = false, prestaged_bwd = false;
+  bool feeds_out_xent = false;
   DevGraph *forward_graph() const;
   DevGraph *backward_graph() const;
   DevGraph *forward_table_graph() const;
diff --git a/parallel-gcn_amd/csrc/k_elementwise.hip b/parallel-gcn_amd/csrc/k_elementwise.hip
--- a/parallel-gcn_amd/csrc/k_elementwise.hip
+++ b/parallel-gcn_amd/csrc/k_elementwise.hip
@@ -2,6 +2,7 @@
 
 #include "common.hpp"
 #include "kernels.hpp"
+#include "lds_dma.hpp"
 #include "mask_draw.hpp"
 #include "peer_sync.hpp"
 #include "softmax_parts.hpp"
@@ -295,7 +296,7 @@
 #else
 #define XST(k) ((void)0)
 #endif
-template <bool FUSED, int CC = 0, int LDC = 0, int KH = 0>
+template <bool FUSED, int CC = 0, int LDC = 0, int KH = 0, bool PART = false>
 __device__ __forceinline__ void xent_tile(float *__restrict__ logits, int ld_rt,
                                                   float *__restrict__ grad,
                                                   const int *__restrict__ truth, int n, int c_rt,
@@ -305,7 +306,8 @@
                                                   const float *__restrict__ W, int ldw,
                                                   float *__restrict__ dH, int lddh,
                                                   float *__restrict__ dWp, const XentTable &tb,
-                                                  const XentFinal &fin) {
+                                                  const XentFinal &fin,
+                                                  const RingPartials &rp = RingPartials{}) {
   extern __shared__ float smem[];
   __shared__ float red[2 * (XT / 64)];
 #ifdef PGCN_XENT_STAMPS
@@ -359,7 +361,20 @@
   if constexpr (FUSED) {
     const long long grow = wrow0 + ii < n ? wrow0 + ii : n - 1;
     const float *hr = H + grow * (long long)ldh;
-    if (4 * gi + 3 < kh && ldh % 4 == 0) {
+    float4 pp[4], pq[4];
+    float ps = 0.0f;
+    if constexpr (PART) {
+      const float4 *pr = rp.partial + grow * 4 + gi;
+#pragma unroll
+      for (int b = 0; b < 4; b++)
+        pp[b] = pr[(long long)min(b, rp.n_blocks - 1) * rp.part_stride * 4];
+      if (rp.n_blocks > 4) {
+#pragma unroll
+        for (int b = 0; b < 4; b++)
+          pq[b] = pr[(long long)min(4 + b, rp.n_blocks - 1) * rp.part_stride * 4];
+      }
+      ps = rp.row_scale[grow];
+    } else if (4 * gi + 3 < kh && ldh % 4 == 0) {
       const float4 h4 = *reinterpret_cast<const float4 *>(hr + 4 * gi);
       ha[0] = h4.x;
       ha[1] = h4.y;
@@ -369,7 +384,7 @@
 #pragma unroll
       for (int t4 = 0; t4 < 4; t4++) ha[t4] = 4 * gi + t4 < kh ? hr[4 * gi + t4] : 0.0f;
     }
-    if (training && dWp) {
+    if (!PART && training && dWp) {
 #pragma unroll
       for (int st = 0; st < 4; st++) {
         const int rloc = 4 * st + gi;
@@ -378,6 +393,38 @@
     }
     for (int k = wv; k < 16; k += XT / 64)
       for (int j = ln; j < ld; j += 64) wt[k * ld + j] = (k < kh && j < c) ? W[(long long)k * ldw + j] : 0.0f;
+    if constexpr (PART) {
+      float4 a = pp[0];
+#pragma unroll
+      for (int b = 1; b < 4; b++)
+        if (b < rp.n_blocks) f4_acc(a, pp[b]);
+      if (rp.n_blocks > 4) {
+#pragma unroll
+        for (int b = 0; b < 4; b++)
+          if (4 + b < rp.n_blocks) f4_acc(a, pq[b]);
+      }
+      a.x *= ps;
+      a.y *= ps;
+      a.z *= ps;
+      a.w *= ps;
+      if (wrow0 + ii < n)
+        *reinterpret_cast<float4 *>(const_cast<float *>(H) + grow * (long long)ldh + 4 * gi) = a;
+      ha[0] = a.x;
+      ha[1] = a.y;
+      ha[2] = a.z;
+      ha[3] = a.w;
+      if (training && dWp) {
+        *reinterpret_cast<float4 *>(L + ii * S + 4 * gi) = a;
+        wave_lds_fence();
+#pragma unroll
+        for (int st = 0; st < 4; st++) {
+          const int rloc = 4 * st + gi;
+          const float x = L[rloc * S + ii];
+          hw[st] = rloc < wrows ? x : 0.0f;
+        }
+        wave_lds_fence();
+      }
+    }
     __syncthreads();
     if (tb_p >= 0) tb_s = tb.scale[tb_p];
     XST(1);
@@ -602,16 +649,23 @@
       int n, int c, int count, int training, float *__restrict__ partials, int write_back,       \
       const float *__restrict__ H, int ldh, int kh, const float *__restrict__ W, int ldw,        \
       float *__restrict__ dH, int lddh, float *__restrict__ dWp, XentTable tb, XentFinal fin
+#define PGCN_XENT_PASS                                                                          \
+  logits, ld, grad, truth, n, c, count, training, partials, write_back, H, ldh, kh, W, ldw, dH,  \
+      lddh, dWp, tb, fin
 __global__ __launch_bounds__(XT) void k_xent_fwd(PGCN_XENT_ARGS) {
-  xent_tile<false>(logits, ld, grad, truth, n, c, count, training, partials, write_back, H, ldh,
-                   kh, W, ldw, dH, lddh, dWp, tb, fin);
+  xent_tile<false>(PGCN_XENT_PASS);
 }
 template <int CC, int LDC, int KH>
 __global__ __launch_bounds__(XT) __attribute__((amdgpu_waves_per_eu(8))) void k_out_xent(
     PGCN_XENT_ARGS) {
-  xent_tile<true, CC, LDC, KH>(logits, ld, grad, truth, n, c, count, training, partials,
-                               write_back, H, ldh, kh, W, ldw, dH, lddh, dWp, tb, fin);
-}
+  xent_tile<true, CC, LDC, KH>(PGCN_XENT_PASS);
+}
+template <int CC, int LDC, int KH>
+__global__ __launch_bounds__(XT) __attribute__((amdgpu_waves_per_eu(8))) void k_out_xent_part(
+    PGCN_XENT_ARGS, RingPartials rp) {
+  xent_tile<true, CC, LDC, KH, true>(PGCN_XENT_PASS, rp);
+}
+#undef PGCN_XENT_PASS
 #undef PGCN_XENT_ARGS
 
 __global__ __launch_bounds__(1024) void k_reduce_scalars(const float *__restrict__ partials,
@@ -902,8 +956,12 @@
 void launch_out_xent(const float *H, int ldh, int kh, const float *W, int ldw, float *logits,
                      int ld, float *grad, const int *truth, int n, int c, int count, int training,
                      float *partials, hipStream_t s, float *dH, int lddh, float *dWp,
-                     const XentTable *tb, const XentFinal *fin) {
+                     const XentTable *tb, const XentFinal *fin, const RingPartials *rp) {
   note_path(KP_OUT_XENT);
+  PGCN_CHECK(!rp || (rp->partial && rp->row_scale && rp->n_blocks >= 1 &&
+                     rp->n_blocks <= kXentMaxPartials && rp->part_stride >= n && kh == 16 &&
+                     ldh % 4 == 0 && ldh >= 16 && H),
+             PGCN_E_INVALID, "out_xent: partials of a 16-column H, at most 8 blocks");
   PGCN_CHECK(!fin || (fin->ticket && fin->part4 && fin->out2 &&
                       (fin->group == 0 || (fin->group > 0 && fin->gticket && fin->gpart4))),
              PGCN_E_INVALID,
@@ -920,7 +978,19 @@
   PGCN_LAUNCH((k_out_xent<__VA_ARGS__>), dim3(xent_blocks(n)), dim3(XT), lds, s, logits, ld, grad, \
               truth, n, c, count, training, partials, 1, H, ldh, kh, W, ldw,                     \
               training ? dH : nullptr, lddh, training ? dWp : nullptr, t, fin ? *fin : XentFinal{})
-  if (c == 41 && ld == 44 && kh == 16)
+  if (rp) {
+    note_path(KP_OUT_XENT_PART);
+#define OUT_XENT_PART(...)                                                                     \
+  PGCN_LAUNCH((k_out_xent_part<__VA_ARGS__>), dim3(xent_blocks(n)), dim3(XT), lds, s, logits, ld, \
+              grad, truth, n, c, count, training, partials, 1, H, ldh, kh, W, ldw,               \
+              training ? dH : nullptr, lddh, training ? dWp : nullptr, t,                        \
+              fin ? *fin : XentFinal{}, *rp)
+    if (c == 41 && ld == 44)
+      OUT_XENT_PART(41, 44, 16);
+    else
+      OUT_XENT_PART(0, 0, 0);
+#undef OUT_XENT_PART
+  } else if (c == 41 && ld == 44 && kh == 16)
     OUT_XENT(41, 44, 16);
   else if (c == 7 && ld == 8 && kh == 16)
     OUT_XENT(7, 8, 16);
diff --git a/parallel-gcn_amd/csrc/k_graphsum_ring.hip b/parallel-gcn_amd/csrc/k_graphsum_ring.hip
--- a/parallel-gcn_amd/csrc/k_graphsum_ring.hip
+++ b/parallel-gcn_amd/csrc/k_graphsum_ring.hip
@@ -439,9 +439,12 @@
 void launch_graphsum_ring(const LdsSchedule &s, const float *in, int ld_in, float *out,
                           int ld_out, float *scratch_in, float *partial, hipStream_t st,
                           const int *col_map, const GsEpilogue *epi, bool prestaged,
-                          const PeerSink *push, hipStream_t tail_st, hipEvent_t fork) {
+                          const PeerSink *push, hipStream_t tail_st, hipEvent_t fork,
+                          RingPartials *stop) {
   note_path(KP_GS_RING);
   PGCN_CHECK(!tail_st || (push && fork), PGCN_E_INVALID, "graphsum_ring: tail stream of a push");
+  PGCN_CHECK(!stop || (!push && (!epi || (epi->mode == 0 && !epi->next_table))), PGCN_E_INVALID,
+             "graphsum_ring: partials handed on have no push and no epilogue");
   PGCN_CHECK(ld_in % 4 == 0 && ld_out % 4 == 0, PGCN_E_INVALID, "graphsum_ring: ld % 4");
   const long long pre = (long long)s.n_cols * 4;
   if (!prestaged)
@@ -464,6 +467,15 @@
   else
     RING_LAUNCH(16, false, 3);
 #undef RING_LAUNCH
+  if (stop) {
+    stop->partial = reinterpret_cast<const float4 *>(partial);
+    stop->part_stride = (long long)s.n_rows;
+    stop->n_blocks = s.n_blocks;
+    stop->row_scale = s.row_scale;
+    PGCN_HIP(hipGetLastError());
+    return;
+  }
+  note_path(KP_GS_COMBINE);
   const GsEpilogue none{};
   const long long post = (long long)s.n_rows * 4;
   if (push) {
@@ -489,4 +501,16 @@
   PGCN_HIP(hipGetLastError());
 }
 
-}
+void launch_ring_combine(const RingPartials &p, int n, float *out, int ld_out, hipStream_t st) {
+  PGCN_CHECK(p.partial && p.row_scale && p.n_blocks >= 1 && p.part_stride >= n && out &&
+                 ld_out % 4 == 0 && ld_out >= 16,
+             PGCN_E_INVALID, "ring_combine: shape");
+  if (n <= 0) return;
+  note_path(KP_GS_COMBINE);
+  PGCN_LAUNCH(k_gs_lds_combine<false>, dim3((unsigned)ceil_div((long long)n * 4, 256)), dim3(256),
+              0, st, p.partial, p.part_stride, p.n_blocks, p.row_scale, n,
+              reinterpret_cast<float4 *>(out), ld_out / 4, GsEpilogue{}, PeerSink{});
+  PGCN_HIP(hipGetLastError());
+}
+
+}
diff --git a/parallel-gcn_amd/csrc/kernels.hpp b/parallel-gcn_amd/csrc/kernels.hpp
--- a/parallel-gcn_amd/csrc/kernels.hpp
+++ b/parallel-gcn_amd/csrc/kernels.hpp
@@ -12,7 +12,8 @@
   KP_XS_NN_RING, KP_XS_TN_RING, KP_XS_NN, KP_XS_TN, KP_GS_RING, KP_GS_GATHER, KP_OUT_XENT,
   KP_GEMM_NN, KP_GEMM_TN, KP_GEMM_NN_W, KP_GEMM_TN_W, KP_GAT_FWD, KP_GAT_BWD, KP_GAT_HEADS,
   KP_SPMM_CSR, KP_SPMM_CSR_DUAL, KP_SPMM_CSC_256, KP_SPMM_CSC_1024, KP_SPMM_TREE_256,
-  KP_SPMM_TREE_1024, KP_LAUNCHES, KP_LINK_FWD, KP_LINK_BWD, KP_COUNT
+  KP_SPMM_TREE_1024, KP_LAUNCHES, KP_LINK_FWD, KP_LINK_BWD, KP_GS_COMBINE, KP_OUT_XENT_PART,
+  KP_COUNT
 };
 void note_path(KernelPath p);
 #define PGCN_LAUNCH(...)                     \
@@ -99,7 +100,8 @@
                           int ld_out, float *scratch_in, float *partial, hipStream_t st,
                           const int *col_map = nullptr, const GsEpilogue *epi = nullptr,
                           bool prestaged = false, const struct PeerSink *push = nullptr,
-                          hipStream_t tail_st = nullptr, hipEvent_t fork = nullptr);
+                          hipStream_t tail_st = nullptr, hipEvent_t fork = nullptr,
+                          struct RingPartials *stop = nullptr);
 void launch_gs_finish(float *y, int ld, int n, int dim, const GsEpilogue &epi, hipStream_t st);
 
 void launch_gemm_nn(int M, int N, int K, const float *A, int lda, const float *B, int ldb,
@@ -340,11 +342,19 @@
   unsigned *gticket = nullptr;
   float4 *gpart4 = nullptr;
 };
+constexpr int kXentMaxPartials = 8;
+struct RingPartials {
+  const float4 *partial = nullptr;
+  long long part_stride = 0;
+  int n_blocks = 0;
+  const float *row_scale = nullptr;
+};
+void launch_ring_combine(const RingPartials &p, int n, float *out, int ld_out, hipStream_t st);
 void launch_out_xent(const float *H, int ldh, int kh, const float *W, int ldw, float *logits,
                      int ld, float *grad, const int *truth, int n, int c, int count, int training,
                      float *partials, hipStream_t s, float *dH = nullptr, int lddh = 0,
                      float *dWp = nullptr, const XentTable *tb = nullptr,
-                     const XentFinal *fin = nullptr);
+                     const XentFinal *fin = nullptr, const RingPartials *rp = nullptr);
 void launch_tn_reduce_blocks(float *partial, int n_blocks, int K, int N, int ldp, float *C, int ldc,
                              hipStream_t s);
 float *tn_defer_blocks(int n_blocks, int K, int N, int ldp, float *C, int ldc);
diff --git a/parallel-gcn_amd/csrc/knobs.cpp b/parallel-gcn_amd/csrc/knobs.cpp
--- a/parallel-gcn_amd/csrc/knobs.cpp
+++ b/parallel-gcn_amd/csrc/knobs.cpp
@@ -60,4 +60,9 @@
   return k;
 }
 
+int &out_xent_fold() {
+  static int on = 1;
+  return on;
 }
+
+}
diff --git a/parallel-gcn_amd/csrc/knobs.hpp b/parallel-gcn_amd/csrc/knobs.hpp
--- a/parallel-gcn_amd/csrc/knobs.hpp
+++ b/parallel-gcn_amd/csrc/knobs.hpp
@@ -49,5 +49,6 @@
 extern const int kKnobCount;
 const KnobRow *find_knob(const char *name);
 Knobs &process_knobs();
+int &out_xent_fold();
 
 }
```

Result: no change. 619.8 (median of 6 runs) (+0.7%).
